# nianticlabs/mickey

Measured on AMD Instinct MI355X. Metric: image pairs/sec (540x720), higher is better.
Workload: dtype bf16

## Files before the change

### include/mickey_hip_dev.h

```cpp
#ifndef MICKEY_HIP_DEV_H
#define MICKEY_HIP_DEV_H

#ifdef __cplusplus
extern "C" {
#endif

int mk_gemm_set_tile(int mode);

int mk_attn_set_mode(int mode);

int mk_dev_mfma_sustained(float* scratch, int workgroups, int iters, int zero_operands, void* stream);

#ifdef __cplusplus
}
#endif
#endif
```

### mickey_amd/_native.py

```python
import ctypes
import os

import torch

from . import build as _build

MK_BF16, MK_F16, MK_F32 = 0, 1, 2
ACT_NONE, ACT_RELU, ACT_GELU = 0, 1, 2

_P, _I, _L, _F, _U = ctypes.c_void_p, ctypes.c_int, ctypes.c_longlong, ctypes.c_float, ctypes.c_ulonglong
_CODES = {"p": _P, "i": _I, "l": _L, "f": _F, "u": _U}

SIGNATURES = {
    "mk_version": ("i", ""),
    "mk_last_error": ("s", ""),
    "mk_preprocess_u8": ("i", "pliiipiip"),
    "mk_gemm": ("i", "pipippiiiiiiip"),
    "mk_gemm_grouped": ("i", "pilpilplpiliiiiiiip"),
    "mk_gemm_ls_residual": ("i", "pipipppiiiiip"),
    "mk_gemm_qkv": ("i", "pipippppiiiifip"),
    "mk_gemm_patch_embed": ("i", "pipipppiiiiip"),
    "mk_gemm_ls_residual_ln": ("i", "pipippppipppiiiiip"),
    "mk_gemm_patch_embed_ln": ("i", "pipipppppiiiiip"),
    "mk_cls_token_ln": ("i", "pppppiiiip"),
    "mk_recentre_split": ("i", "ppplilp"),
    "mk_gemm_ln": ("i", "pipipppfppiiiiiip"),
    "mk_gemm_qkv_ln": ("i", "pipipppfppppiiiifip"),
    "mk_im2col_patch14": ("i", "plliiiipiip"),
    "mk_cls_token": ("i", "pppiiip"),
    "mk_layernorm": ("i", "pippfpiipiiiiiiiiiip"),
    "mk_gemm_ln128": ("i", "pilpilppfpipiiiiiiip"),
    "mk_layernorm_planes": ("i", "pippfppifpiiiiiiiiipp"),
    "mk_flash_attn_fwd": ("i", "ppppiiiiiip"),
    "mk_bordered_rows": ("l", "iii"),
    "mk_conv3x3": ("i", "pliplipilplplpiliiiiiiip"),
    "mk_conv3x3_split": ("i", "pplipplipilplppiliiiiiiffpp"),
    "mk_split_planes": ("i", "plilfpplpp"),
    "mk_gemm_grouped_split": ("i", "ppilpilplppiliiiiiffpp"),
    "mk_posenc_add": ("i", "ppppiiiiiip"),
    "mk_linattn_work_floats": ("l", "iiii"),
    "mk_linattn_kv": ("i", "pppiiiip"),
    "mk_linattn_apply": ("i", "pppiiiiiip"),
    "mk_head_tails": ("i", "pppppppppppiiiiiiiififp"),
    "mk_dual_softmax_work_floats": ("l", "iiii"),
    "mk_dual_softmax": ("i", "ppppfifppppiiiip"),
    "mk_dual_softmax_split_work_floats": ("l", "iii"),
    "mk_dual_softmax_split": ("i", "ppppfifppppiiiip"),
    "mk_sinkhorn_work_floats": ("l", "iii"),
    "mk_sinkhorn": ("i", "ppppfippppiiiip"),
    "mk_dual_softmax_kf": ("i", "ppppfifppppiiiipip"),
    "mk_dual_softmax_split_kf": ("i", "ppppfifppppiiiipip"),
    "mk_sinkhorn_kf": ("i", "ppppfippppiiiipip"),
    "mk_mutual_nn": ("i", "ppppiiip"),
    "mk_dual_softmax_train_work_floats": ("l", "iiii"),
    "mk_dual_softmax_train": ("i", "ppppfppppppiiiiip"),
    "mk_dual_softmax_bwd_work_floats": ("l", "iiii"),
    "mk_dual_softmax_bwd": ("i", "ppppfpppppppppiiiiip"),
    "mk_exprace_topk_work_bytes": ("l", "iiil"),
    "mk_exprace_topk_state_bytes": ("l", "ii"),
    "mk_exprace_topk": ("i", "ppuupppppiiliip"),
    "mk_counter_add": ("i", "pup"),
    "mk_gather_backproject": ("i", "ppppppppppppiiiiip"),
    "mk_gather_backproject_kf": ("i", "ppppppppppppiiiiipip"),
    "mk_gather_backproject_bwd": ("i", "ppppppppppiiiiip"),
    "mk_ransac_hypotheses": ("i", "pppppuupfppppiiilp"),
    "mk_refine_pose": ("i", "pppppfiipppppppiiiip"),
    "mk_pose_finalize": ("i", "ppppip"),
    "mk_train_ransac_masks": ("i", "pppppuupfiipppiiilp"),
    "mk_reinforce_scatter": ("i", "ppppiiilp"),
    "mk_train_tail_fwd": ("i", "pppppppiiiifiifpppp"),
    "mk_train_tail_bwd": ("i", "pppppppiiiifiifppppppp"),
    "mk_train_aggregate_fwd": ("i", "pppiiififfppppp"),
    "mk_train_aggregate_bwd": ("i", "ppiiipp"),
}

DEV_SIGNATURES = {
    "mk_gemm_set_tile": ("i", "i"),
    "mk_attn_set_mode": ("i", "i"),
    "mk_dev_mfma_sustained": ("i", "piiip"),
}

_lib = None
_missing = set()


class MickeyHipError(RuntimeError):
    pass


def lib_path():
    return os.environ.get("MICKEY_HIP_LIB", _build.lib_path())


def load():
    global _lib
    if _lib is not None:
        return _lib
    path = lib_path()
    if not os.path.exists(path):
        raise MickeyHipError("libmickey_hip.so not found at %s -- build it with `python -m mickey_amd.build` "
                             "(mickey_amd has no CPU/ATen fallback)" % path)
    lib = ctypes.CDLL(path)
    for name, (res, args) in list(SIGNATURES.items()) + list(DEV_SIGNATURES.items()):
        try:
            fn = getattr(lib, name)
        except AttributeError:
            _missing.add(name)
            continue
        fn.restype = ctypes.c_char_p if res == "s" else _CODES[res]
        fn.argtypes = [_CODES[c] for c in args]
    _lib = lib
    return lib


def exported_symbols():
    return list(SIGNATURES)


def missing_symbols():
    load()
    return sorted(_missing)


def ptr(t):
    if t is None:
        return None
    if not t.is_cuda:
        raise MickeyHipError("expected a device tensor")
    return t.data_ptr()


def stream():
    return torch.cuda.current_stream().cuda_stream


def dtype_code(dt):
    if dt == torch.bfloat16:
        return MK_BF16
    if dt == torch.float16:
        return MK_F16
    if dt == torch.float32:
        return MK_F32
    raise MickeyHipError("unsupported low-precision dtype %s" % dt)


def call(name, *args):
    lib = load()
    if name in _missing:
        raise MickeyHipError("libmickey_hip.so does not export %s (stale build?)" % name)
    rc = getattr(lib, name)(*args)
    if rc != 0:
        raise MickeyHipError("%s failed (%d): %s" % (name, rc, lib.mk_last_error().decode()))


def query(name, *args):
    return getattr(load(), name)(*args)
```

### mickey_amd/csrc/mk_gemm.hip

```cpp
#include "mk_gemm_common.hpp"

namespace mk {
namespace gemm {
namespace {

template <typename T, int AMODE, int WMF, bool SP = false>
__global__ __launch_bounds__(256, 1) void gemm_kernel(GemmParams p) {
  using V8 = typename Lp<T>::V8;
  constexpr int NWM = 2, NWN = 2;
  constexpr int NW = NWM * NWN, BM = NWM * WMF * 16, BN = NWN * 64;
  constexpr int AJ = BM / 8 / NW, WJ = BN / 8 / NW;
  constexpr int A_BYTES = BM * 128, STAGE_BYTES = (BM + BN) * 128;
  constexpr int NS = WMF == 2 ? 3 : 2;
  constexpr int PIECES = AJ + WJ;
  extern __shared__ __attribute__((aligned(16))) char smem[];

  const int tid = threadIdx.x;
  const int lane = tid & 63;
  const int wave = __builtin_amdgcn_readfirstlane(tid >> 6);
  const int wm = wave / NWN, wn = wave % NWN;
  const int g = blockIdx.y;
  const int ntm = (p.M + BM - 1) / BM, ntn = (p.N + BN - 1) / BN;
  const int nk = p.K / BK;
  const int fr = lane & 15, fg = lane >> 4;

  const int id = xcd_remap(blockIdx.x, ntm * ntn);
  const int m0 = (id / ntn) * BM, n0 = (id % ntn) * BN;
  Stager<T, AMODE, NW, AJ, WJ, SP> st;
  st.init(p, g, m0, n0, wave, lane);
  st.issue(p, smem, smem + A_BYTES, 0);
  if (NS == 3 && nk > 1) st.issue(p, smem + STAGE_BYTES, smem + STAGE_BYTES + A_BYTES, 1);
  float2* lnp = (float2*)(smem + NS * STAGE_BYTES);
  if (AMODE == A_DENSE && p.ln_stats && tid < 2 * BM) ln_params_to_lds<BM, 2 * BM>(p, m0, tid, lnp, p.ln_shift_out != nullptr && n0 == 0);
  f32x4 acc[WMF][4];
#pragma unroll
  for (int i = 0; i < WMF; ++i)
#pragma unroll
    for (int j = 0; j < 4; ++j) acc[i][j] = f32x4{0.f, 0.f, 0.f, 0.f};
  int cur = 0, nxt = NS - 1;
  for (int kt = 0; kt < nk; ++kt) {
    if (NS == 3 && kt + 1 < nk) asm volatile("s_waitcnt vmcnt(%0)" ::"n"(PIECES) : "memory");
    else asm volatile("s_waitcnt vmcnt(0)" ::: "memory");
    asm volatile("s_waitcnt lgkmcnt(0)" ::: "memory");
    __builtin_amdgcn_s_barrier();
    char* nA = smem + nxt * STAGE_BYTES;
    if (kt + NS - 1 < nk) st.issue(p, nA, nA + A_BYTES, kt + NS - 1);
    const char* sA = smem + cur * STAGE_BYTES;
    const char* sW = sA + A_BYTES;
    cur = cur + 1 == NS ? 0 : cur + 1;
    nxt = nxt + 1 == NS ? 0 : nxt + 1;
    if constexpr (SP) {
      V8 wf[2][4], xf[2][WMF];
#pragma unroll
      for (int ks = 0; ks < 2; ++ks) {
#pragma unroll
        for (int i = 0; i < 4; ++i) {
          const int rw = wn * 64 + i * 16 + fr;
          wf[ks][i] = *(const V8*)(sW + rw * 128 + swz8(rw, ks * 4 + fg) * 16);
        }
#pragma unroll
        for (int i = 0; i < WMF; ++i) {
          const int rx = wm * (WMF * 16) + i * 16 + fr;
          xf[ks][i] = *(const V8*)(sA + rx * 128 + swz8(rx, ks * 4 + fg) * 16);
        }
      }
#pragma unroll
      for (int pr = 0; pr < 3; ++pr) {
        if (pr == 2 && p.npass == 2) break;
#pragma unroll
        for (int mi = 0; mi < WMF; ++mi)
#pragma unroll
          for (int ni = 0; ni < 4; ++ni) acc[mi][ni] = Lp<T>::mma16(wf[pr == 1][ni], xf[pr == 2][mi], acc[mi][ni]);
      }
    } else {
#pragma unroll
      for (int ks = 0; ks < 2; ++ks) {
        V8 wf[4], xf[WMF];
#pragma unroll
        for (int i = 0; i < 4; ++i) {
          const int rw = wn * 64 + i * 16 + fr;
          wf[i] = *(const V8*)(sW + rw * 128 + swz8(rw, ks * 4 + fg) * 16);
        }
#pragma unroll
        for (int i = 0; i < WMF; ++i) {
          const int rx = wm * (WMF * 16) + i * 16 + fr;
          xf[i] = *(const V8*)(sA + rx * 128 + swz8(rx, ks * 4 + fg) * 16);
        }
#pragma unroll
        for (int mi = 0; mi < WMF; ++mi)
#pragma unroll
          for (int ni = 0; ni < 4; ++ni) acc[mi][ni] = Lp<T>::mma16(wf[ni], xf[mi], acc[mi][ni]);
      }
    }
  }
  epilogue<T, WMF>(p, acc, m0, n0, wm, wn, lane, g, lnp);
}

template <typename T, int AMODE, int WMF, bool SP = false>
int launch_small(const GemmParams& p, int groups, hipStream_t st) {
  constexpr int BM = 32 * WMF;
  constexpr int LDS = (WMF == 2 ? 3 : 2) * (BM + 128) * 128 + BM * 8;
  static bool attr_done = false;
  if (!attr_done) {
    hipError_t e = hipFuncSetAttribute((const void*)gemm_kernel<T, AMODE, WMF, SP>, hipFuncAttributeMaxDynamicSharedMemorySize, LDS);
    if (e != hipSuccess) {
      mk_set_error("gemm: cannot reserve %d B of LDS: %s", LDS, hipGetErrorString(e));
      return MK_ERR_LAUNCH;
    }
    attr_done = true;
  }
  const int ntm = (p.M + BM - 1) / BM, ntn = (p.N + 127) / 128;
  hipLaunchKernelGGL((gemm_kernel<T, AMODE, WMF, SP>), dim3(ntm * ntn, groups, 1), dim3(256), LDS, st, p);
  MK_CHECK_LAUNCH();
  return MK_OK;
}

int g_num_cus = 0;
int g_band_m = 0;
int g_half_rows = 1;
int g_schedule = 0;

template <int AMODE>
int launch(const GemmParams& p, int groups, int dtype, hipStream_t st) {
  const long long big_tiles = (long long)((p.M + 255) / 256) * ((p.N + 255) / 256) * groups;
  bool big = p.N >= 256 && big_tiles >= 192;
  const long long plmax = p.npass > 1 ? (long long)max(max(p.pl1[0], p.pl1[1]), max(p.pl2[0], p.pl2[1])) / 2 : 0;
  const bool k_ok = p.K >= 2 * BK && (long long)p.M * p.lda + plmax < (1ll << 31) && (long long)p.N * p.ldw < (1ll << 31) &&
                    (AMODE == A_DENSE || bordered_rows(p.M / (p.H * p.Wd), p.H, p.Wd) * (p.C1 > p.C2 ? p.C1 : p.C2) + plmax < (1ll << 31));
  const bool ln_fold = p.ln_stats || p.xh;
  if (dtype == MK_F32) {
    MK_CHECK_ARG(!ln_fold, "gemm: the folded-LayerNorm epilogues exist for 16-bit operands only");
    return launch_f32(p, groups, AMODE, st);
  }
  int sched = g_schedule;
  if (sched == 0) sched = (big && k_ok) ? 7 : 1;
  if (!k_ok) sched = 1;
  if (sched == 7) return launch_pp64(p, groups, dtype, AMODE, st, g_band_m);
  const long long small_tiles = (long long)((p.M + 127) / 128) * ((p.N + 127) / 128) * groups;
  const bool half_rows = g_schedule == 2 || (g_schedule != 1 && g_half_rows && small_tiles < 2 * num_cus() && p.M > 64);
  if (p.npass > 1)
    return half_rows ? launch_small<_Float16, AMODE, 2, true>(p, groups, st) : launch_small<_Float16, AMODE, 4, true>(p, groups, st);
  if (half_rows) return dtype == MK_BF16 ? launch_small<__bf16, AMODE, 2>(p, groups, st) : launch_small<_Float16, AMODE, 2>(p, groups, st);
  return dtype == MK_BF16 ? launch_small<__bf16, AMODE, 4>(p, groups, st) : launch_small<_Float16, AMODE, 4>(p, groups, st);
}

int check_common(const GemmParams& p, int dtype) {
  MK_CHECK_ARG(dtype == MK_BF16 || dtype == MK_F16 || dtype == MK_F32, "gemm: dtype must be MK_BF16, MK_F16 or MK_F32");
  MK_CHECK_ARG(p.M > 0 && p.N > 0 && p.K > 0, "gemm: empty problem M=%d N=%d K=%d", p.M, p.N, p.K);
  const int kt = dtype == MK_F32 ? KT<float> : BK;
  MK_CHECK_ARG(p.K % kt == 0, "gemm: K=%d must be a multiple of %d", p.K, kt);
  MK_CHECK_ARG(p.N % 4 == 0, "gemm: N=%d must be a multiple of 4", p.N);
  MK_CHECK_ARG(p.ldw % 8 == 0 && p.ldw >= p.K, "gemm: ldw=%d must be >= K and a multiple of 8", p.ldw);
  MK_CHECK_ARG(p.A && p.W, "gemm: null operand");
  return MK_OK;
}

}

int num_cus() {
  if (g_num_cus == 0) {
    int dev = 0, n = 0;
    if (hipGetDevice(&dev) != hipSuccess || hipDeviceGetAttribute(&n, hipDeviceAttributeMultiprocessorCount, dev) != hipSuccess || n <= 0)
      n = 256;
    g_num_cus = n;
  }
  return g_num_cus;
}

}
}

using namespace mk;
using namespace mk::gemm;

extern "C" {

int mk_gemm_set_tile(int mode) {
  if (mode >= 400 && mode < 464) {
    g_band_m = mode - 400;
    return MK_OK;
  }
  if (mode >= 464 && mode < 496) {
    g_band_m = -(mode - 464);
    return MK_OK;
  }
  if (mode == 500 || mode == 501) {
    g_half_rows = mode - 500;
    return MK_OK;
  }
  if (mode >= 600 && mode <= 602) {
    g_pp64_persist = mode - 600;
    return MK_OK;
  }
  MK_CHECK_ARG(mode == 0 || mode == 1 || mode == 2 || mode == 7,
               "mk_gemm_set_tile: unknown mode %d (0 automatic, 1 128x128, 2 64x128, 7 8-wave ping-pong)", mode);
  g_schedule = mode;
  return MK_OK;
}

int mk_gemm(const void* A, int lda, const void* W, int ldw, const float* bias, void* out, int ldc, int M, int N, int K,
            int act, int out_is_f32, int dtype, mk_stream_t stream) {
  GemmParams p = {};
  p.A = A; p.W = W; p.M = M; p.N = N; p.K = K; p.lda = lda; p.ldw = ldw;
  p.epi = MK_EPI_STORE; p.act = act; p.bias = bias; p.ldc = ldc;
  if (out_is_f32) p.out_f32 = (float*)out; else p.out_lp = out;
  if (int e = check_common(p, dtype)) return e;
  MK_CHECK_ARG(lda % 8 == 0 && lda >= K && ldc % 4 == 0 && ldc >= N && out, "mk_gemm: bad lda/ldc/out");
  return launch<A_DENSE>(p, 1, dtype, (hipStream_t)stream);
}

int mk_gemm_grouped(const void* A, int lda, long long strideA, const void* W, int ldw, long long strideW, const float* bias,
                    long long strideBias, void* out, int ldc, long long strideOut, int groups, int M, int N, int K, int act,
                    int out_is_f32, int dtype, mk_stream_t stream) {
  GemmParams p = {};
  p.A = A; p.W = W; p.M = M; p.N = N; p.K = K; p.lda = lda; p.ldw = ldw;
  p.strideA_g = strideA; p.strideW_g = strideW; p.strideBias_g = strideBias; p.strideOut_g = strideOut;
  p.epi = MK_EPI_STORE; p.act = act; p.bias = bias; p.ldc = ldc;
  if (out_is_f32) p.out_f32 = (float*)out; else p.out_lp = out;
  if (int e = check_common(p, dtype)) return e;
  MK_CHECK_ARG(groups > 0 && lda % 8 == 0 && lda >= K && ldc % 4 == 0 && ldc >= N && out, "mk_gemm_grouped: bad args");
  return launch<A_DENSE>(p, groups, dtype, (hipStream_t)stream);
}

int mk_gemm_ls_residual(const void* A, int lda, const void* W, int ldw, const float* bias, const float* gamma, float* x,
                        int ldx, int M, int N, int K, int dtype, mk_stream_t stream) {
  GemmParams p = {};
  p.A = A; p.W = W; p.M = M; p.N = N; p.K = K; p.lda = lda; p.ldw = ldw;
  p.epi = MK_EPI_LS_RESIDUAL; p.bias = bias; p.gamma = gamma; p.out_f32 = x; p.ldc = ldx;
  if (int e = check_common(p, dtype)) return e;
  MK_CHECK_ARG(bias && gamma && x && lda % 8 == 0 && lda >= K && ldx % 4 == 0 && ldx >= N, "mk_gemm_ls_residual: bad args");
  return launch<A_DENSE>(p, 1, dtype, (hipStream_t)stream);
}

int mk_gemm_qkv(const void* A, int lda, const void* W, int ldw, const float* bias, void* q, void* k, void* vt, int nimg,
                int ntok, int ntok_pad, int heads, float qscale, int dtype, mk_stream_t stream) {
  GemmParams p = {};
  const int D = heads * 64;
  p.A = A; p.W = W; p.M = nimg * ntok; p.N = 3 * D; p.K = D; p.lda = lda; p.ldw = ldw;
  p.epi = MK_EPI_QKV; p.bias = bias; p.q = q; p.k = k; p.vt = vt;
  p.ntok = ntok; p.ntok_pad = ntok_pad; p.heads = heads; p.qscale = qscale;
  if (int e = check_common(p, dtype)) return e;
  MK_CHECK_ARG(bias && q && k && vt && ntok_pad % 64 == 0 && ntok_pad >= ntok && lda % 8 == 0 && lda >= D, "mk_gemm_qkv: bad args");
  return launch<A_DENSE>(p, 1, dtype, (hipStream_t)stream);
}

int mk_gemm_patch_embed(const void* A, int lda, const void* W, int ldw, const float* bias, const float* pos, float* x,
                        int nimg, int npatch, int D, int K, int dtype, mk_stream_t stream) {
  GemmParams p = {};
  p.A = A; p.W = W; p.M = nimg * npatch; p.N = D; p.K = K; p.lda = lda; p.ldw = ldw;
  p.epi = MK_EPI_PATCH; p.bias = bias; p.pos = pos; p.npatch = npatch; p.out_f32 = x; p.ldc = D;
  if (int e = check_common(p, dtype)) return e;
  MK_CHECK_ARG(bias && pos && x && lda % 8 == 0 && lda >= K, "mk_gemm_patch_embed: bad args");
  return launch<A_DENSE>(p, 1, dtype, (hipStream_t)stream);
}


static int ln_consumer_args(GemmParams& p, const float* colsum, const float* stats, float eps, float* shift_out, const char* who) {
  MK_CHECK_ARG(colsum && stats && p.bias, "%s: colsum, stats and bias are required", who);
  MK_CHECK_ARG(p.lda == p.K, "%s: the normalised width is K: lda must equal K", who);
  p.ln_colsum = colsum; p.ln_stats = stats; p.ln_nslot = p.K / 64; p.ln_eps = eps; p.ln_shift_out = shift_out;
  return MK_OK;
}

int mk_gemm_ln(const void* A, int lda, const void* W, int ldw, const float* bias, const float* colsum, const float* stats,
               float eps, float* shift_out, void* out, int ldc, int M, int N, int K, int act, int dtype, mk_stream_t stream) {
  GemmParams p = {};
  p.A = A; p.W = W; p.M = M; p.N = N; p.K = K; p.lda = lda; p.ldw = ldw;
  p.epi = MK_EPI_STORE; p.act = act; p.bias = bias; p.ldc = ldc; p.out_lp = out;
  if (int e = check_common(p, dtype)) return e;
  MK_CHECK_ARG(lda % 8 == 0 && ldc % 4 == 0 && ldc >= N && out && (act == MK_ACT_NONE || act == MK_ACT_GELU), "mk_gemm_ln: bad args");
  if (int e = ln_consumer_args(p, colsum, stats, eps, shift_out, "mk_gemm_ln")) return e;
  return launch<A_DENSE>(p, 1, dtype, (hipStream_t)stream);
}

int mk_gemm_qkv_ln(const void* A, int lda, const void* W, int ldw, const float* bias, const float* colsum, const float* stats,
                   float eps, float* shift_out, void* q, void* k, void* vt, int nimg, int ntok, int ntok_pad, int heads,
                   float qscale, int dtype, mk_stream_t stream) {
  GemmParams p = {};
  const int D = heads * 64;
  p.A = A; p.W = W; p.M = nimg * ntok; p.N = 3 * D; p.K = D; p.lda = lda; p.ldw = ldw;
  p.epi = MK_EPI_QKV; p.bias = bias; p.q = q; p.k = k; p.vt = vt;
  p.ntok = ntok; p.ntok_pad = ntok_pad; p.heads = heads; p.qscale = qscale;
  if (int e = check_common(p, dtype)) return e;
  MK_CHECK_ARG(q && k && vt && ntok_pad % 64 == 0 && ntok_pad >= ntok && lda % 8 == 0, "mk_gemm_qkv_ln: bad args");
  if (int e = ln_consumer_args(p, colsum, stats, eps, shift_out, "mk_gemm_qkv_ln")) return e;
  return launch<A_DENSE>(p, 1, dtype, (hipStream_t)stream);
}

int mk_gemm_ls_residual_ln(const void* A, int lda, const void* W, int ldw, const float* bias, const float* gamma, void* xh,
                           void* xl, int ldxs, float* stats, const float* shift_in, float* x_f32_out, int ldx, int M, int N,
                           int K, int dtype, mk_stream_t stream) {
  GemmParams p = {};
  p.A = A; p.W = W; p.M = M; p.N = N; p.K = K; p.lda = lda; p.ldw = ldw;
  p.epi = MK_EPI_LS_RESIDUAL; p.bias = bias; p.gamma = gamma; p.out_f32 = x_f32_out; p.ldc = ldx;
  p.xh = xh; p.xl = xl; p.ldxs = ldxs; p.stats_out = stats; p.nslot_out = N / 64; p.ln_shift_in = shift_in;
  if (int e = check_common(p, dtype)) return e;
  MK_CHECK_ARG(bias && gamma && lda % 8 == 0 && lda >= K, "mk_gemm_ls_residual_ln: bad args");
  MK_CHECK_ARG(xh && xl && N % 64 == 0 && ldxs % 8 == 0 && ldxs >= N, "mk_gemm_ls_residual_ln: xh / xl / N %% 64");
  MK_CHECK_ARG(x_f32_out ? (ldx % 4 == 0 && ldx >= N) : stats != nullptr, "mk_gemm_ls_residual_ln: stats, or x_f32_out with ldx");
  return launch<A_DENSE>(p, 1, dtype, (hipStream_t)stream);
}

int mk_gemm_patch_embed_ln(const void* A, int lda, const void* W, int ldw, const float* bias, const float* pos, void* xh,
                           void* xl, float* stats, int nimg, int npatch, int D, int K, int dtype, mk_stream_t stream) {
  GemmParams p = {};
  p.A = A; p.W = W; p.M = nimg * npatch; p.N = D; p.K = K; p.lda = lda; p.ldw = ldw;
  p.epi = MK_EPI_PATCH; p.bias = bias; p.pos = pos; p.npatch = npatch; p.ldc = D;
  p.xh = xh; p.xl = xl; p.ldxs = D; p.stats_out = stats; p.nslot_out = D / 64;
  if (int e = check_common(p, dtype)) return e;
  MK_CHECK_ARG(bias && pos && lda % 8 == 0 && lda >= K, "mk_gemm_patch_embed_ln: bad args");
  MK_CHECK_ARG(xh && xl && stats && D % 64 == 0, "mk_gemm_patch_embed_ln: xh / xl / stats / D %% 64");
  return launch<A_DENSE>(p, 1, dtype, (hipStream_t)stream);
}

long long mk_bordered_rows(int nimg, int H, int Wd) { return bordered_rows(nimg, H, Wd); }

int mk_conv3x3(const void* in1, long long stride_in1, int C1, const void* in2, long long stride_in2, int C2, const void* W,
               int ldw, long long strideW, const float* bias, long long strideBias, const void* resid, long long strideResid,
               void* out, int Cout, long long strideOut, int groups, int nimg, int H, int Wd, int act, int out_kind, int dtype,
               mk_stream_t stream) {
  GemmParams p = {};
  p.A = in1; p.A2 = in2; p.W = W;
  p.M = nimg * H * Wd; p.N = Cout; p.K = 9 * C1 + (in2 ? C2 : 0);
  p.ldw = ldw; p.strideA_g = stride_in1; p.strideA2_g = stride_in2; p.strideW_g = strideW;
  p.strideBias_g = strideBias; p.strideOut_g = strideOut;
  p.H = H; p.Wd = Wd; p.C1 = C1; p.C2 = in2 ? C2 : 0;
  p.epi = MK_EPI_STORE; p.act = act; p.bias = bias; p.ldc = Cout; p.resid_lp = resid; p.strideResid_g = strideResid;
  if (out_kind == MK_CONV_OUT_F32) p.out_f32 = (float*)out; else p.out_lp = out;
  p.bord_out = out_kind == MK_CONV_OUT_BORDERED;
  if (int e = check_common(p, dtype)) return e;
  MK_CHECK_ARG(C1 % (dtype == MK_F32 ? 32 : BK) == 0 && (!in2 || C2 % (dtype == MK_F32 ? 32 : BK) == 0),
               "mk_conv3x3: channel counts must be multiples of the K tile (%d)", dtype == MK_F32 ? 32 : BK);
  MK_CHECK_ARG(out && groups > 0 && nimg > 0 && H > 0 && Wd > 0 && out_kind >= 0 && out_kind <= 2, "mk_conv3x3: bad args");
  return launch<A_CONV3>(p, groups, dtype, (hipStream_t)stream);
}

namespace {
__global__ __launch_bounds__(256) void split_planes_kernel(const float* __restrict__ src, long long rows, int cols4, long long ld_src4,
                                                           float scale, uint2* __restrict__ hi, uint2* __restrict__ lo, long long ld_dst4, int* sat_flag) {
  const long long t = blockIdx.x * 256LL + threadIdx.x;
  if (t >= rows * cols4) return;
  const long long r = t / cols4;
  const int c = (int)(t - r * cols4);
  const long long i = r * ld_dst4 + c;
  const f32x4 x = __builtin_nontemporal_load((const f32x4*)src + r * ld_src4 + c) * scale;
  f16x4 h, l;
#pragma unroll
  for (int e = 0; e < 4; ++e) {
    const float v = sat16(x[e], sat_flag);
    h[e] = (_Float16)v;
    l[e] = (_Float16)(v - (float)h[e]);
  }
  hi[i] = __builtin_bit_cast(uint2, h);
  lo[i] = __builtin_bit_cast(uint2, l);
}
}

int mk_split_planes(const float* src, long long rows, int cols, long long ld_src, float scale, void* hi, void* lo,
                    long long ld_dst, int* sat_flag, mk_stream_t stream) {
  MK_CHECK_ARG(src && hi && lo && rows > 0 && cols > 0 && cols % 4 == 0 && ld_src % 4 == 0 && ld_dst % 4 == 0 && ld_src >= cols &&
                   ld_dst >= cols, "mk_split_planes: cols / ld_src / ld_dst must be multiples of 4 and ld >= cols");
  MK_CHECK_ARG((((uintptr_t)src | (uintptr_t)hi * 2 | (uintptr_t)lo * 2) & 15) == 0, "mk_split_planes: src must be 16-byte, planes 8-byte aligned");
  const long long n4 = rows * (cols / 4);
  hipLaunchKernelGGL(split_planes_kernel, dim3((unsigned)((n4 + 255) / 256)), dim3(256), 0, (hipStream_t)stream, src, rows, cols / 4,
                     ld_src / 4, scale, (uint2*)hi, (uint2*)lo, ld_dst / 4, sat_flag);
  MK_CHECK_LAUNCH();
  return MK_OK;
}

static int split_source(const void* hi, const void* lo, const void*& base, unsigned (&pl)[2], const char* who) {
  const uintptr_t h = (uintptr_t)hi, l = (uintptr_t)lo, b = h < l ? h : l;
  MK_CHECK_ARG((h - b) < (1ull << 31) && (l - b) < (1ull << 31) && ((h | l) & 15) == 0,
               "%s: the (hi, lo) planes of a source must be 16-byte aligned and lie within 2 GiB of each other", who);
  base = (const void*)b;
  pl[0] = (unsigned)(h - b);
  pl[1] = (unsigned)(l - b);
  return MK_OK;
}

int mk_gemm_grouped_split(const void* A_hi, const void* A_lo, int lda, long long strideA, const void* W, int ldw, long long strideW,
                          const float* bias, long long strideBias, void* out, void* out_lo, int ldc, long long strideOut, int groups,
                          int M, int N, int K, int act, float acc_scale, float plane_scale, int* sat_flag, mk_stream_t stream) {
  GemmParams p = {};
  MK_CHECK_ARG(A_hi && A_lo, "mk_gemm_grouped_split: null plane");
  if (int e = split_source(A_hi, A_lo, p.A, p.pl1, "mk_gemm_grouped_split")) return e;
  p.W = W; p.M = M; p.N = N; p.K = 2 * K; p.lda = lda; p.ldw = ldw;
  p.npass = 3; p.acc_scale = acc_scale;
  p.strideA_g = strideA; p.strideW_g = strideW; p.strideBias_g = strideBias; p.strideOut_g = strideOut;
  p.epi = MK_EPI_STORE; p.act = act; p.bias = bias; p.ldc = ldc;
  if (out_lo) { p.out_lp = out; p.out_lo = out_lo; p.plane_scale = plane_scale; p.sat_flag = sat_flag; } else { p.out_f32 = (float*)out; }
  if (int e = check_common(p, MK_F16)) return e;
  MK_CHECK_ARG(out && groups > 0 && K % 32 == 0 && lda % 8 == 0 && lda >= K && ldc % 4 == 0 && ldc >= N,
               "mk_gemm_grouped_split: bad args (K must be a multiple of 32)");
  return launch<A_DENSE>(p, groups, MK_F16, (hipStream_t)stream);
}

int mk_conv3x3_split(const void* in1_hi, const void* in1_lo, long long stride_in1, int C1, const void* in2_hi, const void* in2_lo,
                     long long stride_in2, int C2, const void* W, int ldw, long long strideW, const float* bias,
                     long long strideBias, void* out, void* out_lo, int Cout, long long strideOut, int groups, int nimg, int H,
                     int Wd, int act, int out_bordered, float acc_scale, float plane_scale, int* sat_flag, mk_stream_t stream) {
  GemmParams p = {};
  const bool hi_only = in1_hi && !in1_lo;
  MK_CHECK_ARG(in1_hi && (hi_only ? (!in2_hi && !in2_lo) : (!in2_hi == !in2_lo)),
               "mk_conv3x3_split: every source needs both planes (in1_lo == NULL = an all-zero lo plane: then without in2)");
  if (int e = split_source(in1_hi, hi_only ? in1_hi : in1_lo, p.A, p.pl1, "mk_conv3x3_split")) return e;
  if (in2_hi) {
    if (int e = split_source(in2_hi, in2_lo, p.A2, p.pl2, "mk_conv3x3_split")) return e;
  }
  p.W = W;
  p.npass = hi_only ? 2 : 3; p.acc_scale = acc_scale;
  p.M = nimg * H * Wd; p.N = Cout; p.K = 2 * (9 * C1 + (in2_hi ? C2 : 0));
  p.ldw = ldw; p.strideA_g = stride_in1; p.strideA2_g = stride_in2; p.strideW_g = strideW;
  p.strideBias_g = strideBias; p.strideOut_g = strideOut;
  p.H = H; p.Wd = Wd; p.C1 = C1; p.C2 = in2_hi ? C2 : 0;
  p.epi = MK_EPI_STORE; p.act = act; p.bias = bias; p.ldc = Cout;
  if (out_lo) { p.out_lp = out; p.out_lo = out_lo; p.plane_scale = plane_scale; p.sat_flag = sat_flag; } else { p.out_f32 = (float*)out; }
  p.bord_out = out_bordered ? 1 : 0;
  if (int e = check_common(p, MK_F16)) return e;
  MK_CHECK_ARG(C1 % 32 == 0 && (!in2_hi || C2 % 32 == 0), "mk_conv3x3_split: channel counts must be multiples of 32");
  MK_CHECK_ARG(out && groups > 0 && nimg > 0 && H > 0 && Wd > 0, "mk_conv3x3_split: bad args");
  return launch<A_CONV3>(p, groups, MK_F16, (hipStream_t)stream);
}

}
```

### mickey_amd/csrc/mk_gemm_common.hpp

```cpp
#pragma once
#include "mk_common.hpp"

namespace mk {
namespace gemm {

constexpr int BK = 64;
template <typename T> constexpr int EPC = 16 / (int)sizeof(T);
template <typename T> constexpr int KT = 128 / (int)sizeof(T);

enum AMode { A_DENSE = 0, A_CONV3 = 1 };

struct GemmParams {
  const void* A;
  const void* A2;
  const void* W;
  int M, N, K, lda, ldw;
  long long strideA_g, strideA2_g, strideW_g;
  int H, Wd, C1, C2;
  int bord_out;
  unsigned pl1[2], pl2[2];
  int npass;
  float acc_scale;
  void* out_lo;
  float plane_scale;
  int* sat_flag;
  int epi;
  int act;
  const float* bias;
  const float* gamma;
  long long strideBias_g;
  float* out_f32;
  void* out_lp;
  int ldc;
  long long strideOut_g;
  const void* resid_lp;
  long long strideResid_g;
  void* q;
  void* k;
  void* vt;
  int ntok, ntok_pad, heads;
  float qscale;
  const float* pos;
  int npatch;
  void* xh;
  void* xl;
  int ldxs;
  float* stats_out;
  int nslot_out;
  const float* ln_stats;
  const float* ln_colsum;
  int ln_nslot;
  float ln_eps;
  float* ln_shift_out;
  const float* ln_shift_in;
};

__device__ __forceinline__ void quad_stats(const f32x4& x, float& s, float& q) {
  s = x[0];
  s += x[1];
  s += x[2];
  s += x[3];
  q = __builtin_fmaf(x[0], x[0], 0.0f);
  q = __builtin_fmaf(x[1], x[1], q);
  q = __builtin_fmaf(x[2], x[2], q);
  q = __builtin_fmaf(x[3], x[3], q);
}

__device__ __forceinline__ float row16_sum(float v) {
#define MK_DPP_ADD(ctrl) v += __builtin_bit_cast(float, __builtin_amdgcn_update_dpp(0, __builtin_bit_cast(int, v), ctrl, 0xf, 0xf, true))
  MK_DPP_ADD(0xB1);
  MK_DPP_ADD(0x4E);
  MK_DPP_ADD(0x141);
  MK_DPP_ADD(0x140);
#undef MK_DPP_ADD
  return v;
}

typedef __attribute__((ext_vector_type(4))) unsigned u32x4;
struct LnRowLoads16 {
  u32x4 v[4];
  __device__ __forceinline__ void issue(const GemmParams& p, int m0, int tid) {
    const int wave = tid >> 6, lane = tid & 63;
    const long long last = (long long)p.M * 128 - 16;
#pragma unroll
    for (int j = 0; j < 4; ++j) {
      long long off = ((long long)(m0 + wave * 32 + j * 8) * 128) + lane * 16;
      off = off < last ? off : last;
      const char* a = (const char*)p.ln_stats + off;
      asm volatile("global_load_dwordx4 %0, %1, off" : "=v"(v[j]) : "v"(a) : "memory");
    }
  }
  template <int YOUNGER>
  __device__ __forceinline__ void finish(const GemmParams& p, int tid, float2* prm, int m0 = 0, bool publish = false) {
    asm volatile("s_waitcnt vmcnt(%4)" : "+v"(v[0]), "+v"(v[1]), "+v"(v[2]), "+v"(v[3]) : "n"(YOUNGER) : "memory");
    const int wave = tid >> 6, lane = tid & 63;
#pragma unroll
    for (int j = 0; j < 4; ++j) {
      const f32x4 f = __builtin_bit_cast(f32x4, v[j]);
      float s = f[0] + f[2], q = f[1] + f[3];
#define MK_DPP_ADD(x, ctrl) x += __builtin_bit_cast(float, __builtin_amdgcn_update_dpp(0, __builtin_bit_cast(int, x), ctrl, 0xf, 0xf, true))
      MK_DPP_ADD(s, 0xB1);  MK_DPP_ADD(q, 0xB1);
      MK_DPP_ADD(s, 0x4E);  MK_DPP_ADD(q, 0x4E);
      MK_DPP_ADD(s, 0x141); MK_DPP_ADD(q, 0x141);
#undef MK_DPP_ADD
      const double mean = (double)s * (1.0 / 1024.0);
      double var = (double)q * (1.0 / 1024.0) - mean * mean;
      var = var > 0.0 ? var : 0.0;
      const float rstd = 1.0f / sqrtf((float)var + p.ln_eps);
      if ((lane & 7) == 0) {
        const int r = wave * 32 + j * 8 + (lane >> 3);
        prm[r] = make_float2(rstd, -(float)mean * rstd);
        if (publish && m0 + r < p.M) p.ln_shift_out[m0 + r] = (float)mean;
      }
    }
  }
};

struct LnRowDma16 {
  template <int J0>
  __device__ __forceinline__ static void issue(const GemmParams& p, int m0, int wave, int lane, char* stage_lds) {
    const long long last = (long long)p.M * 128 - 16;
#pragma unroll
    for (int j = J0; j < J0 + 2; ++j) {
      const long long base = (long long)(m0 + wave * 32 + j * 8) * 128;
      long long off = base + lane * 16;
      off = off < last ? off : last;
      glds16_sv((const char*)p.ln_stats, (unsigned)off, stage_lds + (wave * 2 + (j - J0)) * 1024);
    }
  }
  template <int J0>
  __device__ __forceinline__ static void finish(const GemmParams& p, int wave, int lane, float2* prm, const char* stage_lds, int m0,
                                                bool publish) {
#pragma unroll
    for (int j = J0; j < J0 + 2; ++j) {
      const f32x4 f = *(const f32x4*)(stage_lds + (wave * 2 + (j - J0)) * 1024 + lane * 16);
      float s = f[0] + f[2], q = f[1] + f[3];
#define MK_DPP_ADD(x, ctrl) x += __builtin_bit_cast(float, __builtin_amdgcn_update_dpp(0, __builtin_bit_cast(int, x), ctrl, 0xf, 0xf, true))
      MK_DPP_ADD(s, 0xB1);  MK_DPP_ADD(q, 0xB1);
      MK_DPP_ADD(s, 0x4E);  MK_DPP_ADD(q, 0x4E);
      MK_DPP_ADD(s, 0x141); MK_DPP_ADD(q, 0x141);
#undef MK_DPP_ADD
      const double mean = (double)s * (1.0 / 1024.0);
      double var = (double)q * (1.0 / 1024.0) - mean * mean;
      var = var > 0.0 ? var : 0.0;
      const float rstd = 1.0f / sqrtf((float)var + p.ln_eps);
      if ((lane & 7) == 0) {
        const int r = wave * 32 + j * 8 + (lane >> 3);
        prm[r] = make_float2(rstd, -(float)mean * rstd);
        if (publish && m0 + r < p.M) p.ln_shift_out[m0 + r] = (float)mean;
      }
    }
  }
};

struct ShiftLoad {
  float v;
  __device__ __forceinline__ void issue(const GemmParams& p, int m0, int tid, int BM) {
    v = 0.f;
    if (p.ln_shift_in && tid < BM) {
      int m = m0 + tid;
      m = m < p.M ? m : p.M - 1;
      const float* a = p.ln_shift_in + m;
      asm volatile("global_load_dword %0, %1, off" : "=v"(v) : "v"(a) : "memory");
    }
  }
  template <int YOUNGER>
  __device__ __forceinline__ void finish(int tid, int BM, float* shl) {
    if constexpr (YOUNGER >= 0)
      asm volatile("s_waitcnt vmcnt(%1)" : "+v"(v) : "n"(YOUNGER) : "memory");
    else
      asm volatile("" : "+v"(v) : : "memory");
    if (tid < BM) shl[tid] = v;
  }
};

template <int BM, int NT>
__device__ __forceinline__ void ln_params_to_lds(const GemmParams& p, int m0, int tid, float2* prm, bool publish = false) {
  static_assert(NT == 2 * BM, "two threads per row");
  const int r = tid >> 1, h = tid & 1;
  int m = m0 + r;
  m = m < p.M ? m : p.M - 1;
  const float2* st = (const float2*)p.ln_stats + (long long)m * p.ln_nslot;
  float s, q;
  if (p.ln_nslot <= 16) {
    float2 v[8];
#pragma unroll
    for (int j = 0; j < 8; ++j) v[j] = 8 * h + j < p.ln_nslot ? st[8 * h + j] : make_float2(0.f, 0.f);
    const float s01 = v[0].x + v[1].x, s23 = v[2].x + v[3].x, s45 = v[4].x + v[5].x, s67 = v[6].x + v[7].x;
    const float q01 = v[0].y + v[1].y, q23 = v[2].y + v[3].y, q45 = v[4].y + v[5].y, q67 = v[6].y + v[7].y;
    s = (s01 + s23) + (s45 + s67);
    q = (q01 + q23) + (q45 + q67);
  } else {
    const int per = (p.ln_nslot + 1) >> 1;
    const int lo = h * per, hi = min(p.ln_nslot, lo + per);
    s = q = 0.f;
    for (int i0 = lo; i0 < hi; i0 += 8) {
      float2 v[8];
#pragma unroll
      for (int j = 0; j < 8; ++j) v[j] = i0 + j < hi ? st[i0 + j] : make_float2(0.f, 0.f);
#pragma unroll
      for (int j = 0; j < 8; ++j) {
        s += v[j].x;
        q += v[j].y;
      }
    }
  }
  s += __shfl_xor(s, 1, 64);
  q += __shfl_xor(q, 1, 64);
  const double invn = 1.0 / (64.0 * p.ln_nslot);
  const double mean = (double)s * invn;
  double var = (double)q * invn - mean * mean;
  var = var > 0.0 ? var : 0.0;
  const float rstd = 1.0f / sqrtf((float)var + p.ln_eps);
  if (h == 0) {
    prm[r] = make_float2(rstd, -(float)mean * rstd);
    if (publish && m0 + r < p.M) p.ln_shift_out[m0 + r] = (float)mean;
  }
}

template <typename T>
__device__ __forceinline__ T to_lp(float v) { return (T)v; }

template <typename T>
__device__ __forceinline__ f32x4 unpack4(uint2 u);
template <>
__device__ __forceinline__ f32x4 unpack4<__bf16>(uint2 u) {
  return f32x4{__builtin_bit_cast(float, u.x << 16), __builtin_bit_cast(float, u.x & 0xffff0000u),
               __builtin_bit_cast(float, u.y << 16), __builtin_bit_cast(float, u.y & 0xffff0000u)};
}
template <>
__device__ __forceinline__ f32x4 unpack4<_Float16>(uint2 u) {
  const f16x4 h = __builtin_bit_cast(f16x4, u);
  return f32x4{(float)h[0], (float)h[1], (float)h[2], (float)h[3]};
}
template <>
__device__ __forceinline__ f32x4 unpack4<float>(uint2) { return f32x4{0.f, 0.f, 0.f, 0.f}; }
template <typename T>
__device__ __forceinline__ uint2 pack4(f32x4 v) {
  typename Lp<T>::V4 o;
#pragma unroll
  for (int e = 0; e < 4; ++e) o[e] = to_lp<T>(v[e]);
  if constexpr (sizeof(T) == 2) return __builtin_bit_cast(uint2, o);
  else return uint2{0u, 0u};
}

__device__ __forceinline__ int vperm(int t) { return (t & ~12) | ((t & 4) << 1) | ((t & 8) >> 1); }

template <typename T, int AMODE, int NW, int AJ, int WJ, bool SP = false>
struct Stager {
  const T* A;
  const T* A2;
  const T* wrow[WJ];
  long long aoff[AJ];
  int wave, srow, sp;

  __device__ __forceinline__ void init(const GemmParams& p, int g, int m0, int n0, int wave_, int lane) {
    wave = wave_;
    srow = lane >> 3;
    sp = lane & 7;
    A = (const T*)p.A + (long long)g * p.strideA_g;
    A2 = p.A2 ? (const T*)p.A2 + (long long)g * p.strideA2_g : nullptr;
    const T* W = (const T*)p.W + (long long)g * p.strideW_g;
#pragma unroll
    for (int j = 0; j < WJ; ++j) {
      const int r = (wave * WJ + j) * 8 + srow;
      int n = n0 + r;
      n = n < p.N ? n : p.N - 1;
      wrow[j] = W + (long long)n * p.ldw + swz8(r, sp) * EPC<T>;
    }
#pragma unroll
    for (int j = 0; j < AJ; ++j) {
      const int r = (wave * AJ + j) * 8 + srow;
      int m = m0 + r;
      m = m < p.M ? m : p.M - 1;
      const int c = swz8(r, sp);
      if (AMODE == A_DENSE) aoff[j] = SP ? (long long)m * p.lda + (c & 3) * EPC<T> + (long long)(((c >> 2) ? p.pl1[1] : p.pl1[0]) / sizeof(T))
                                         : (long long)m * p.lda + c * EPC<T>;
      else aoff[j] = bordered_row(m, p.H, p.Wd);
    }
  }

  __device__ __forceinline__ void issue(const GemmParams& p, char* sA, char* sW, int kt) const {
    const int k0 = kt * KT<T>;
    const int ka = SP ? kt * (KT<T> / 2) : k0;
    if (AMODE == A_DENSE) {
#pragma unroll
      for (int j = 0; j < AJ; ++j) glds16(A + aoff[j] + ka, sA + (wave * AJ + j) * 1024);
    } else {
      const int kc = 9 * p.C1;
      const T* const s1 = A;
      const T* const s2 = A2;
      const T* src;
      int cs, c0, shift = 0;
      unsigned plh, pll;
      if (ka < kc) {
        const int tap = ka / p.C1;
        c0 = ka - tap * p.C1;
        shift = (tap / 3 - 1) * (p.Wd + 1) + tap % 3 - 1;
        src = s1;
        cs = p.C1;
        plh = p.pl1[0];
        pll = p.pl1[1];
      } else {
        c0 = ka - kc;
        src = s2;
        cs = p.C2;
        plh = p.pl2[0];
        pll = p.pl2[1];
      }
#pragma unroll
      for (int j = 0; j < AJ; ++j) {
        const int r = (wave * AJ + j) * 8 + srow;
        const int c = swz8(r, sp);
        if (SP) glds16(src + (aoff[j] + shift) * cs + c0 + (c & 3) * EPC<T> + (long long)(((c >> 2) ? pll : plh) / sizeof(T)), sA + (wave * AJ + j) * 1024);
        else glds16(src + (aoff[j] + shift) * cs + c0 + c * EPC<T>, sA + (wave * AJ + j) * 1024);
      }
    }
#pragma unroll
    for (int j = 0; j < WJ; ++j) glds16(wrow[j] + k0, sW + (wave * WJ + j) * 1024);
  }
};

template <typename T, int WMF, int EPI, int ACT, bool HAS_BIAS, bool LN = false, bool SPLIT = false>
__device__ __forceinline__ void epilogue_impl(const GemmParams& p, f32x4 (&acc)[WMF][4], int m0, int n0, int wm, int wn, int lane,
                                              int g, const float2* lnp = nullptr) {
  using V4 = typename Lp<T>::V4;
  const int fr = lane & 15, fg = lane >> 4;
  const float* bias = HAS_BIAS ? p.bias + (long long)g * p.strideBias_g : nullptr;
  const int nb = n0 + wn * 64 + fg * 4;
  f32x4 bv[4], cs[4];
#pragma unroll
  for (int ni = 0; ni < 4; ++ni) {
    const int n = nb + ni * 16;
    bv[ni] = (HAS_BIAS && n < p.N) ? *(const f32x4*)(bias + n) : f32x4{0.f, 0.f, 0.f, 0.f};
    cs[ni] = (LN && n < p.N) ? *(const f32x4*)(p.ln_colsum + n) : f32x4{0.f, 0.f, 0.f, 0.f};
  }
  const bool fin = SPLIT && EPI == MK_EPI_LS_RESIDUAL && p.out_f32 != nullptr;
#pragma unroll
  for (int mi = 0; mi < WMF; ++mi) {
    const int m = m0 + wm * (WMF * 16) + mi * 16 + fr;
    if (SPLIT) {
      const bool mok = m < p.M;
      long long xrow = m;
      int tok1 = 0;
      if (EPI == MK_EPI_PATCH) {
        const int img = m / p.npatch;
        tok1 = 1 + (m - img * p.npatch);
        xrow = (long long)img * (p.npatch + 1) + tok1;
      }
      const float shv = (EPI == MK_EPI_LS_RESIDUAL && p.ln_shift_in && mok) ? p.ln_shift_in[m] : 0.f;
      float s4[4] = {0.f, 0.f, 0.f, 0.f}, q4[4] = {0.f, 0.f, 0.f, 0.f};
#pragma unroll
      for (int ni = 0; ni < 4; ++ni) {
        const int n = nb + ni * 16;
        if (!(mok && n < p.N)) continue;
        f32x4 v = acc[mi][ni] + bv[ni];
        T* ph = (T*)p.xh + xrow * p.ldxs + n;
        T* pl = (T*)p.xl + xrow * p.ldxs + n;
        if (EPI == MK_EPI_LS_RESIDUAL) {
          const f32x4 gm = *(const f32x4*)(p.gamma + n);
          const V4 h = *(const V4*)ph, l = *(const V4*)pl;
          f32x4 r;
#pragma unroll
          for (int e = 0; e < 4; ++e) r[e] = (float)h[e] + (float)l[e];
          r += gm * v;
          r -= shv;
          v = r;
        } else {
          v += *(const f32x4*)(p.pos + (long long)tok1 * p.N + n);
        }
        if (fin) {
          *(f32x4*)(p.out_f32 + xrow * p.ldc + n) = v;
          continue;
        }
        V4 oh, ol;
#pragma unroll
        for (int e = 0; e < 4; ++e) {
          oh[e] = to_lp<T>(v[e]);
          ol[e] = to_lp<T>(v[e] - (float)oh[e]);
        }
        quad_stats(v, s4[ni], q4[ni]);
        *(V4*)ph = oh;
        *(V4*)pl = ol;
      }
#pragma unroll
      for (int ni = 0; ni < 4; ++ni) {
        s4[ni] += __shfl_xor(s4[ni], 16, 64);
        q4[ni] += __shfl_xor(q4[ni], 16, 64);
        s4[ni] += __shfl_xor(s4[ni], 32, 64);
        q4[ni] += __shfl_xor(q4[ni], 32, 64);
      }
      const float ssum = (s4[0] + s4[1]) + (s4[2] + s4[3]), qsum = (q4[0] + q4[1]) + (q4[2] + q4[3]);
      if (!fin && fg == 0 && mok && n0 + wn * 64 < p.N)
        ((float2*)p.stats_out)[xrow * p.nslot_out + ((n0 + wn * 64) >> 6)] = make_float2(ssum, qsum);
      continue;
    }
    if (m >= p.M) continue;
    float2 prm = make_float2(1.f, 0.f);
    if (LN) prm = lnp[wm * (WMF * 16) + mi * 16 + fr];
    int img = 0, tok = 0;
    if (EPI == MK_EPI_QKV) {
      img = m / p.ntok;
      tok = m - img * p.ntok;
    } else if (EPI == MK_EPI_PATCH) {
      img = m / p.npatch;
      tok = m - img * p.npatch;
    }
    const long long brow = (EPI == MK_EPI_STORE && p.H > 0) ? bordered_row(m, p.H, p.Wd) : (long long)m;
#pragma unroll
    for (int ni = 0; ni < 4; ++ni) {
      const int n = nb + ni * 16;
      if (n >= p.N) continue;
      f32x4 v = acc[mi][ni];
      if (EPI == MK_EPI_STORE && p.npass > 1) {
        const float sc = p.acc_scale;
#pragma unroll
        for (int e = 0; e < 4; ++e) v[e] *= sc;
      }
      if (LN) v = v * prm.x + (cs[ni] * prm.y + bv[ni]);
      else if (HAS_BIAS) v += bv[ni];
      if (EPI == MK_EPI_STORE) {
        if (p.resid_lp) {
          const V4 r = *(const V4*)((const T*)p.resid_lp + (long long)g * p.strideResid_g + brow * p.ldc + n);
#pragma unroll
          for (int e = 0; e < 4; ++e) v[e] += (float)r[e];
        }
        if (ACT == MK_ACT_RELU) {
#pragma unroll
          for (int e = 0; e < 4; ++e) v[e] = fmaxf(v[e], 0.f);
        } else if (ACT == MK_ACT_GELU) {
          v = gelu_erf4(v);
        }
        if (p.out_lo) {
          const float ps = p.plane_scale;
          f16x4 oh, ol;
#pragma unroll
          for (int e = 0; e < 4; ++e) {
            const float sv = sat16(v[e] * ps, p.sat_flag);
            oh[e] = (_Float16)sv;
            ol[e] = (_Float16)(sv - (float)oh[e]);
          }
          const long long o = (long long)g * p.strideOut_g + (p.bord_out ? brow : (long long)m) * p.ldc + n;
          *(f16x4*)((_Float16*)p.out_lp + o) = oh;
          *(f16x4*)((_Float16*)p.out_lo + o) = ol;
        } else if (p.out_f32) {
          *(f32x4*)(p.out_f32 + (long long)g * p.strideOut_g + (p.bord_out ? brow : (long long)m) * p.ldc + n) = v;
        } else {
          V4 o;
#pragma unroll
          for (int e = 0; e < 4; ++e) o[e] = to_lp<T>(v[e]);
          *(V4*)((T*)p.out_lp + (long long)g * p.strideOut_g + (p.bord_out ? brow : (long long)m) * p.ldc + n) = o;
        }
      } else if (EPI == MK_EPI_LS_RESIDUAL) {
        float* x = p.out_f32 + (long long)m * p.ldc + n;
        const f32x4 gm = *(const f32x4*)(p.gamma + n);
        f32x4 r = *(const f32x4*)x;
        r += gm * v;
        *(f32x4*)x = r;
      } else if (EPI == MK_EPI_PATCH) {
        const f32x4 pe = *(const f32x4*)(p.pos + (long long)(1 + tok) * p.N + n);
        *(f32x4*)(p.out_f32 + ((long long)img * (p.npatch + 1) + 1 + tok) * p.ldc + n) = v + pe;
      } else {
        const int D = p.heads * 64;
        const int which = n / D;
        const int rem = n - which * D;
        const int head = rem >> 6, d = rem & 63;
        const long long hb = (long long)img * p.heads + head;
        if (which == 2) {
          T* dst = (T*)p.vt + (hb * 64 + d) * p.ntok_pad + vperm(tok);
#pragma unroll
          for (int e = 0; e < 4; ++e) dst[(long long)e * p.ntok_pad] = to_lp<T>(v[e]);
        } else {
          if (which == 0) { const float qs = p.qscale; _Pragma("unroll") for (int e = 0; e < 4; ++e) v[e] *= qs; }
          V4 o;
#pragma unroll
          for (int e = 0; e < 4; ++e) o[e] = to_lp<T>(v[e]);
          T* base = (T*)(which == 0 ? p.q : p.k);
          *(V4*)(base + (hb * p.ntok_pad + tok) * 64 + d) = o;
        }
      }
    }
  }
}

template <typename T, int WMF>
__device__ __forceinline__ void epilogue(const GemmParams& p, f32x4 (&acc)[WMF][4], int m0, int n0, int wm, int wn, int lane,
                                         int g, const float2* lnp = nullptr) {
  if (p.xh) {
    if (p.epi == MK_EPI_PATCH) epilogue_impl<T, WMF, MK_EPI_PATCH, MK_ACT_NONE, true, false, true>(p, acc, m0, n0, wm, wn, lane, g);
    else epilogue_impl<T, WMF, MK_EPI_LS_RESIDUAL, MK_ACT_NONE, true, false, true>(p, acc, m0, n0, wm, wn, lane, g);
    return;
  }
  if (p.ln_stats) {
    if (p.epi == MK_EPI_QKV) epilogue_impl<T, WMF, MK_EPI_QKV, MK_ACT_NONE, true, true>(p, acc, m0, n0, wm, wn, lane, g, lnp);
    else if (p.act == MK_ACT_GELU) epilogue_impl<T, WMF, MK_EPI_STORE, MK_ACT_GELU, true, true>(p, acc, m0, n0, wm, wn, lane, g, lnp);
    else epilogue_impl<T, WMF, MK_EPI_STORE, MK_ACT_NONE, true, true>(p, acc, m0, n0, wm, wn, lane, g, lnp);
    return;
  }
  switch (p.epi) {
    case MK_EPI_LS_RESIDUAL: epilogue_impl<T, WMF, MK_EPI_LS_RESIDUAL, MK_ACT_NONE, true>(p, acc, m0, n0, wm, wn, lane, g); break;
    case MK_EPI_QKV: epilogue_impl<T, WMF, MK_EPI_QKV, MK_ACT_NONE, true>(p, acc, m0, n0, wm, wn, lane, g); break;
    case MK_EPI_PATCH: epilogue_impl<T, WMF, MK_EPI_PATCH, MK_ACT_NONE, true>(p, acc, m0, n0, wm, wn, lane, g); break;
    default:
      if (!p.bias) {
        if (p.act == MK_ACT_RELU) epilogue_impl<T, WMF, MK_EPI_STORE, MK_ACT_RELU, false>(p, acc, m0, n0, wm, wn, lane, g);
        else if (p.act == MK_ACT_GELU) epilogue_impl<T, WMF, MK_EPI_STORE, MK_ACT_GELU, false>(p, acc, m0, n0, wm, wn, lane, g);
        else epilogue_impl<T, WMF, MK_EPI_STORE, MK_ACT_NONE, false>(p, acc, m0, n0, wm, wn, lane, g);
      } else {
        if (p.act == MK_ACT_RELU) epilogue_impl<T, WMF, MK_EPI_STORE, MK_ACT_RELU, true>(p, acc, m0, n0, wm, wn, lane, g);
        else if (p.act == MK_ACT_GELU) epilogue_impl<T, WMF, MK_EPI_STORE, MK_ACT_GELU, true>(p, acc, m0, n0, wm, wn, lane, g);
        else epilogue_impl<T, WMF, MK_EPI_STORE, MK_ACT_NONE, true>(p, acc, m0, n0, wm, wn, lane, g);
      }
  }
}

template <typename T, int EPI, int ACT, bool HAS_BIAS, bool LN = false, bool SPLIT = false, bool FIN = false, bool CONV = false>
__device__ __forceinline__ void epilogue_lds_impl(const GemmParams& p, f32x4 (&acc)[8][4], char* wl0, char* wl1, int m0, int n0, int wm,
                                                  int wn, int lane, int g, const float2* lnp = nullptr) {
  using V4 = typename Lp<T>::V4;
  using V8 = typename Lp<T>::V8;
  const int fr = lane & 15, fg = lane >> 4;
  const float* bias = HAS_BIAS ? p.bias + (long long)g * p.strideBias_g : nullptr;
  const int nw = n0 + wn * 64;
  const int mw = m0 + wm * 128;
  int img0 = 0, tok0 = 0;
  if (EPI == MK_EPI_QKV) {
    img0 = mw / p.ntok;
    tok0 = mw - img0 * p.ntok;
  }
  auto img_tok = [&](int r, int& img, int& tok) {
    if (p.ntok >= 128) {
      const int t = tok0 + r;
      const bool wrap = t >= p.ntok;
      img = img0 + (wrap ? 1 : 0);
      tok = wrap ? t - p.ntok : t;
    } else {
      const int m = mw + r;
      img = m / p.ntok;
      tok = m - img * p.ntok;
    }
  };
  f32x4 bv[4], cs[4];
#pragma unroll
  for (int ni = 0; ni < 4; ++ni) {
    const int n = nw + fg * 4 + ni * 16;
    bv[ni] = (HAS_BIAS && n < p.N) ? *(const f32x4*)(bias + n) : f32x4{0.f, 0.f, 0.f, 0.f};
    cs[ni] = (LN && n < p.N) ? *(const f32x4*)(p.ln_colsum + n) : f32x4{0.f, 0.f, 0.f, 0.f};
  }
  float2 prm[8];
#pragma unroll
  for (int mi = 0; mi < 8; ++mi) prm[mi] = LN ? lnp[wm * 128 + mi * 16 + fr] : make_float2(1.f, 0.f);
  const bool lp_out = EPI == MK_EPI_QKV || (EPI == MK_EPI_STORE && !p.out_f32 && !p.out_lo);
  if (lp_out) {
    int which = 0, head = 0;
    if (EPI == MK_EPI_QKV) {
      const int D = p.heads * 64;
      which = nw / D;
      head = (nw - which * D) >> 6;
      if (which == 2) {
#pragma unroll
        for (int mi = 0; mi < 8; ++mi) {
          const int m = mw + mi * 16 + fr;
          if (m >= p.M) continue;
          int img, tok;
          img_tok(mi * 16 + fr, img, tok);
          const long long hb = (long long)img * p.heads + head;
#pragma unroll
          for (int ni = 0; ni < 4; ++ni) {
            const f32x4 v = LN ? acc[mi][ni] * prm[mi].x + (cs[ni] * prm[mi].y + bv[ni]) : acc[mi][ni] + bv[ni];
            T* dst = (T*)p.vt + (hb * 64 + ni * 16 + fg * 4) * p.ntok_pad + vperm(tok);
#pragma unroll
            for (int e = 0; e < 4; ++e) dst[(long long)e * p.ntok_pad] = to_lp<T>(v[e]);
          }
        }
        return;
      }
    }
    const int rr = lane >> 3, c = lane & 7;
    const int n = nw + c * 8;
    const bool bord = CONV && p.bord_out;
    BorderedRow bw;
    if (bord) bw.init(mw + rr, p.H, p.Wd);
#pragma unroll
    for (int h = 0; h < 2; ++h) {
#pragma unroll
      for (int mq = 0; mq < 4; ++mq) {
        const int mi = h * 4 + mq;
        const int r = mi * 16 + fr;
        char* wrow = (mq < 2 ? wl0 : wl1) + ((mq & 1) * 16 + fr) * 128;
        const long long rrow = (CONV && p.resid_lp) ? bordered_row(min(mw + r, p.M - 1), p.H, p.Wd) : 0;
#pragma unroll
        for (int ni = 0; ni < 4; ++ni) {
          f32x4 v = acc[mi][ni];
          if (LN) v = v * prm[mi].x + (cs[ni] * prm[mi].y + bv[ni]);
          else if (HAS_BIAS) v += bv[ni];
          if (EPI == MK_EPI_QKV) {
            if (which == 0) { const float qs = p.qscale; _Pragma("unroll") for (int e = 0; e < 4; ++e) v[e] *= qs; }
          } else {
            if (CONV && p.resid_lp) {
              const int m = mw + r, n2 = nw + fg * 4 + ni * 16;
              if (m < p.M && n2 < p.N) {
                const V4 rs = *(const V4*)((const T*)p.resid_lp + (long long)g * p.strideResid_g + rrow * p.ldc + n2);
#pragma unroll
                for (int e = 0; e < 4; ++e) v[e] += (float)rs[e];
              }
            }
            if (ACT == MK_ACT_RELU) {
#pragma unroll
              for (int e = 0; e < 4; ++e) v[e] = fmaxf(v[e], 0.f);
            } else if (ACT == MK_ACT_GELU) {
              v = gelu_erf4(v);
            }
          }
          V4 o;
#pragma unroll
          for (int e = 0; e < 4; ++e) o[e] = to_lp<T>(v[e]);
          const int cc = ni * 2 + (fg >> 1);
          *(V4*)(wrow + ((cc ^ (fr & 7)) << 4) + (fg & 1) * 8) = o;
        }
      }
#pragma unroll
      for (int i8 = 0; i8 < 8; ++i8) {
        const int it = h * 8 + i8;
        const int r = it * 8 + rr;
        const int m = mw + r;
        const V8 val = *(const V8*)((i8 < 4 ? wl0 : wl1) + ((i8 & 3) * 8 + rr) * 128 + ((c ^ (rr & 7)) << 4));
        const int extra = bord ? bw.extra : 0;
        if (bord) bw.step(8, p.H, p.Wd);
        if (m >= p.M || n >= p.N) continue;
        T* dst;
        if (EPI == MK_EPI_QKV) {
          int img, tok;
          img_tok(r, img, tok);
          dst = (T*)(which == 0 ? p.q : p.k) + (((long long)img * p.heads + head) * p.ntok_pad + tok) * 64 + c * 8;
        } else {
          dst = (T*)p.out_lp + (long long)g * p.strideOut_g + ((long long)m + extra) * p.ldc + n;
        }
        if (n + 8 <= p.N) {
          *(V8*)dst = val;
        } else {
          V4 lo;
#pragma unroll
          for (int e = 0; e < 4; ++e) lo[e] = val[e];
          *(V4*)dst = lo;
        }
      }
    }
  } else {
    const int rr = lane >> 4, c = lane & 15;
    const int n = nw + c * 4;
    f32x4 gm = f32x4{0.f, 0.f, 0.f, 0.f};
    if (EPI == MK_EPI_LS_RESIDUAL && n < p.N) gm = *(const f32x4*)(p.gamma + n);
    f32x4 bvd = f32x4{0.f, 0.f, 0.f, 0.f};
    if (SPLIT && HAS_BIAS && n < p.N) bvd = *(const f32x4*)(bias + n);
    f32x4 xr[2][SPLIT ? 1 : 16];
    uint2 xh[2][SPLIT ? 16 : 1], xl[2][SPLIT ? 16 : 1];
    const unsigned lane_off = (unsigned)rr * (unsigned)p.ldxs + (unsigned)n;
    unsigned lane_off_st = lane_off;
    asm volatile("" : "+v"(lane_off_st));
    auto plane_row = [&](void* plane, int half, int it) -> T* {
      return (T*)plane + (long long)(mw + half * 64 + it * 4) * p.ldxs;
    };
    __amdgpu_buffer_rsrc_t rs_h, rs_l;
    unsigned voff_b = 0;
    if constexpr (SPLIT && EPI == MK_EPI_LS_RESIDUAL && sizeof(T) == 2) {
      rs_h = __builtin_amdgcn_make_buffer_rsrc(p.xh, 0, 0x7fffffff, 0x00020000);
      rs_l = __builtin_amdgcn_make_buffer_rsrc(p.xl, 0, 0x7fffffff, 0x00020000);
      voff_b = lane_off * 2u;
    }
    auto soff_b = [&](int half, int it) -> unsigned {
      return (unsigned)(mw + half * 64 + it * 4) * (unsigned)p.ldxs * 2u;
    };
    typedef unsigned u32x2_t __attribute__((ext_vector_type(2)));
    auto preload = [&](int half, int it0 = 0, int it1 = 16) {
      if (EPI != MK_EPI_LS_RESIDUAL) return;
#pragma unroll
      for (int it = 0; it < 16; ++it) {
        if (it < it0 || it >= it1) continue;
        const int m = mw + half * 64 + it * 4 + rr;
        const bool ok = SPLIT || (m < p.M && n < p.N);
        if constexpr (SPLIT && EPI == MK_EPI_LS_RESIDUAL && sizeof(T) == 2) {
          const u32x2_t a = __builtin_amdgcn_raw_buffer_load_b64(rs_h, voff_b, soff_b(half, it), 0);
          const u32x2_t b = __builtin_amdgcn_raw_buffer_load_b64(rs_l, voff_b, soff_b(half, it), 0);
          xh[half][it] = uint2{a[0], a[1]};
          xl[half][it] = uint2{b[0], b[1]};
        } else if (SPLIT) {
          xh[half][it] = ok ? *(const uint2*)(plane_row(p.xh, half, it) + lane_off) : uint2{0u, 0u};
          xl[half][it] = ok ? *(const uint2*)(plane_row(p.xl, half, it) + lane_off) : uint2{0u, 0u};
        } else {
          xr[half][it] = ok ? *(const f32x4*)(p.out_f32 + (long long)m * p.ldc + n) : f32x4{0.f, 0.f, 0.f, 0.f};
        }
      }
    };
    auto stageq = [&](int half, int sub) {
#pragma unroll
      for (int m2 = 0; m2 < 2; ++m2) {
        const int mi = sub * 2 + m2;
        const int r = mi * 16 + fr;
        char* wrow = (m2 == 0 ? wl0 : wl1) + fr * 256;
        const long long rrow = (CONV && p.resid_lp) ? bordered_row(min(mw + half * 64 + r, p.M - 1), p.H, p.Wd) : 0;
#pragma unroll
        for (int ni = 0; ni < 4; ++ni) {
          f32x4 v = acc[half * 4 + mi][ni];
          if (EPI == MK_EPI_STORE && p.npass > 1) {
            const float sc = p.acc_scale;
#pragma unroll
            for (int e = 0; e < 4; ++e) v[e] *= sc;
          }
          if (HAS_BIAS && !SPLIT) v += bv[ni];
          if (EPI == MK_EPI_STORE) {
            if (CONV && p.resid_lp) {
              const int m = mw + half * 64 + r, nn = nw + fg * 4 + ni * 16;
              if (m < p.M && nn < p.N) {
                const V4 rs = *(const V4*)((const T*)p.resid_lp + (long long)g * p.strideResid_g + rrow * p.ldc + nn);
#pragma unroll
                for (int e = 0; e < 4; ++e) v[e] += (float)rs[e];
              }
            }
            if (ACT == MK_ACT_RELU) {
#pragma unroll
              for (int e = 0; e < 4; ++e) v[e] = fmaxf(v[e], 0.f);
            } else if (ACT == MK_ACT_GELU) {
              v = gelu_erf4(v);
            }
          }
          const int cw = ni * 4 + fg;
          *(f32x4*)(wrow + ((cw ^ fr) << 4)) = v;
        }
      }
    };
    constexpr bool fin = FIN;
    auto emit_row = [&](long long xrow, T* dh, T* dl, f32x4 x, bool ok, unsigned soff = 0xffffffffu) {
      float ssum = 0.f, qsum = 0.f;
      if (ok) {
        const uint2 oh = pack4<T>(x);
        const uint2 ol = pack4<T>(x - unpack4<T>(oh));
        quad_stats(x, ssum, qsum);
        if constexpr (SPLIT && EPI == MK_EPI_LS_RESIDUAL && sizeof(T) == 2) {
          __builtin_amdgcn_raw_buffer_store_b64(u32x2_t{oh.x, oh.y}, rs_h, voff_b, soff, 0);
          __builtin_amdgcn_raw_buffer_store_b64(u32x2_t{ol.x, ol.y}, rs_l, voff_b, soff, 0);
        } else {
          *(uint2*)dh = oh;
          *(uint2*)dl = ol;
        }
      }
      ssum = row16_sum(ssum);
      qsum = row16_sum(qsum);
      if (ok && c == 0) ((float2*)p.stats_out)[xrow * p.nslot_out + (nw >> 6)] = make_float2(ssum, qsum);
    };
    auto drain = [&](int half, int it0 = 0, int it1 = 16) {
      const bool bordf = CONV && p.bord_out;
      BorderedRow bwf;
      if (bordf) bwf.init(mw + half * 64 + it0 * 4 + rr, p.H, p.Wd);
#pragma unroll
      for (int it = 0; it < 16; ++it) {
        if (it < it0 || it >= it1) continue;
        const int r = it * 4 + rr;
        const int m = mw + half * 64 + r;
        const int extraf = bordf ? bwf.extra : 0;
        if (bordf) bwf.step(4, p.H, p.Wd);
        f32x4 val = *(const f32x4*)(((it & 4) ? wl1 : wl0) + ((it & 3) * 4 + rr) * 256 + ((c ^ ((it & 3) * 4 + rr)) << 4));
        if (SPLIT) val += bvd;
        const bool ok = SPLIT || (m < p.M && n < p.N);
        if (!ok) continue;
        if (EPI == MK_EPI_LS_RESIDUAL) {
          f32x4 x;
          if (SPLIT) {
            x = unpack4<T>(xh[half][it]) + unpack4<T>(xl[half][it]);
          } else {
            x = xr[half][it];
          }
          x += gm * val;
          if (SPLIT) x -= ((const float*)lnp)[wm * 128 + half * 64 + r];
          if (!SPLIT || fin) {
            if (ok) *(f32x4*)(p.out_f32 + (long long)m * p.ldc + n) = x;
          } else {
            if constexpr (sizeof(T) == 2) emit_row(m, nullptr, nullptr, x, ok, soff_b(half, it));
            else emit_row(m, plane_row(p.xh, half, it) + lane_off_st, plane_row(p.xl, half, it) + lane_off_st, x, ok);
          }
        } else if (EPI == MK_EPI_PATCH) {
          const int mc = ok ? m : 0;
          const int img = mc / p.npatch, tok = mc - img * p.npatch;
          const long long xrow = (long long)img * (p.npatch + 1) + 1 + tok;
          f32x4 x = val;
          if (ok) x += *(const f32x4*)(p.pos + (long long)(1 + tok) * p.N + n);
          if (SPLIT) emit_row(xrow, (T*)p.xh + xrow * p.ldxs + n, (T*)p.xl + xrow * p.ldxs + n, x, ok);
          else if (ok) *(f32x4*)(p.out_f32 + xrow * p.ldc + n) = x;
        } else if (EPI == MK_EPI_STORE && p.out_lo) {
          const float ps = p.plane_scale;
          f16x4 oh, ol;
#pragma unroll
          for (int e = 0; e < 4; ++e) {
            const float sv = sat16(val[e] * ps, p.sat_flag);
            oh[e] = (_Float16)sv;
            ol[e] = (_Float16)(sv - (float)oh[e]);
          }
          const long long o = (long long)g * p.strideOut_g + ((long long)m + extraf) * p.ldc + n;
          *(f16x4*)((_Float16*)p.out_lp + o) = oh;
          *(f16x4*)((_Float16*)p.out_lo + o) = ol;
        } else {
          *(f32x4*)(p.out_f32 + (long long)g * p.strideOut_g + ((long long)m + extraf) * p.ldc + n) = val;
        }
      }
    };
    if (SPLIT && !FIN && EPI == MK_EPI_LS_RESIDUAL) {
      preload(0, 0, 16);
      stageq(0, 0);
      drain(0, 0, 8);
      preload(1, 0, 8);
      stageq(0, 1);
      drain(0, 8, 16);
      preload(1, 8, 16);
      stageq(1, 0);
      drain(1, 0, 8);
      stageq(1, 1);
      drain(1, 8, 16);
    } else {
      preload(0);
      stageq(0, 0);
      drain(0, 0, 8);
      stageq(0, 1);
      preload(1);
      drain(0, 8, 16);
      stageq(1, 0);
      drain(1, 0, 8);
      stageq(1, 1);
      drain(1, 8, 16);
    }
  }
}

template <typename T, int KIND, bool CONV = false, int BN = 256>
__device__ __forceinline__ void epilogue_lds(const GemmParams& p, f32x4 (&acc)[8][4], char* wl0, char* wl1, int m0, int n0, int wm,
                                             int wn, int lane, int g, const float2* lnp = nullptr) {
  if constexpr (KIND == 2 || KIND == 3) {
    const bool interior = m0 + 256 <= p.M && n0 + BN <= p.N;
    if (KIND == 3) {
      if (interior) epilogue_lds_impl<T, MK_EPI_LS_RESIDUAL, MK_ACT_NONE, true, false, true, true>(p, acc, wl0, wl1, m0, n0, wm, wn, lane, g, lnp);
      else epilogue_impl<T, 8, MK_EPI_LS_RESIDUAL, MK_ACT_NONE, true, false, true>(p, acc, m0, n0, wm, wn, lane, g);
    } else if (p.epi == MK_EPI_PATCH) {
      if (interior) epilogue_lds_impl<T, MK_EPI_PATCH, MK_ACT_NONE, true, false, true>(p, acc, wl0, wl1, m0, n0, wm, wn, lane, g);
      else epilogue_impl<T, 8, MK_EPI_PATCH, MK_ACT_NONE, true, false, true>(p, acc, m0, n0, wm, wn, lane, g);
    } else {
      if (interior) epilogue_lds_impl<T, MK_EPI_LS_RESIDUAL, MK_ACT_NONE, true, false, true, false>(p, acc, wl0, wl1, m0, n0, wm, wn, lane, g, lnp);
      else epilogue_impl<T, 8, MK_EPI_LS_RESIDUAL, MK_ACT_NONE, true, false, true>(p, acc, m0, n0, wm, wn, lane, g);
    }
  } else if constexpr (KIND == 1) {
#if defined(MK_LN_ABL) && MK_LN_ABL == 2
    constexpr bool LNE = false;
#else
    constexpr bool LNE = true;
#endif
    if (p.epi == MK_EPI_QKV) epilogue_lds_impl<T, MK_EPI_QKV, MK_ACT_NONE, true, LNE>(p, acc, wl0, wl1, m0, n0, wm, wn, lane, g, lnp);
    else if (p.act == MK_ACT_GELU) epilogue_lds_impl<T, MK_EPI_STORE, MK_ACT_GELU, true, LNE>(p, acc, wl0, wl1, m0, n0, wm, wn, lane, g, lnp);
    else epilogue_lds_impl<T, MK_EPI_STORE, MK_ACT_NONE, true, LNE>(p, acc, wl0, wl1, m0, n0, wm, wn, lane, g, lnp);
  } else {
    switch (CONV ? MK_EPI_STORE : p.epi) {
      case MK_EPI_LS_RESIDUAL: epilogue_lds_impl<T, MK_EPI_LS_RESIDUAL, MK_ACT_NONE, true>(p, acc, wl0, wl1, m0, n0, wm, wn, lane, g); break;
      case MK_EPI_QKV: epilogue_lds_impl<T, MK_EPI_QKV, MK_ACT_NONE, true>(p, acc, wl0, wl1, m0, n0, wm, wn, lane, g); break;
      case MK_EPI_PATCH: epilogue_lds_impl<T, MK_EPI_PATCH, MK_ACT_NONE, true>(p, acc, wl0, wl1, m0, n0, wm, wn, lane, g); break;
      default:
        if (!p.bias) {
          if (p.act == MK_ACT_RELU) epilogue_lds_impl<T, MK_EPI_STORE, MK_ACT_RELU, false, false, false, false, CONV>(p, acc, wl0, wl1, m0, n0, wm, wn, lane, g);
          else if (!CONV && p.act == MK_ACT_GELU) epilogue_lds_impl<T, MK_EPI_STORE, MK_ACT_GELU, false>(p, acc, wl0, wl1, m0, n0, wm, wn, lane, g);
          else epilogue_lds_impl<T, MK_EPI_STORE, MK_ACT_NONE, false, false, false, false, CONV>(p, acc, wl0, wl1, m0, n0, wm, wn, lane, g);
        } else {
          if (p.act == MK_ACT_RELU) epilogue_lds_impl<T, MK_EPI_STORE, MK_ACT_RELU, true, false, false, false, CONV>(p, acc, wl0, wl1, m0, n0, wm, wn, lane, g);
          else if (!CONV && p.act == MK_ACT_GELU) epilogue_lds_impl<T, MK_EPI_STORE, MK_ACT_GELU, true>(p, acc, wl0, wl1, m0, n0, wm, wn, lane, g);
          else epilogue_lds_impl<T, MK_EPI_STORE, MK_ACT_NONE, true, false, false, false, CONV>(p, acc, wl0, wl1, m0, n0, wm, wn, lane, g);
        }
    }
  }
}

__device__ __forceinline__ void pp_tile_coords(int id, int ntm, int ntn, int PP_GM, int& tm, int& tn) {
  if (PP_GM < 0) {
    const int ng = -PP_GM;
    const int grp = id / (ntm * ng);
    const int rem = id - grp * (ntm * ng);
    const int gn = min(ng, ntn - grp * ng);
    tm = rem / gn;
    tn = grp * ng + rem - tm * gn;
    return;
  }
  const int band = id / (PP_GM * ntn);
  const int rem = id - band * (PP_GM * ntn);
  const int gm = min(PP_GM, ntm - band * PP_GM);
  tm = band * PP_GM + rem % gm;
  tn = rem / gm;
}

int num_cus();
extern int g_pp64_persist;
int launch_pp64(const GemmParams& p, int groups, int dtype, int amode, hipStream_t st, int band_m);
int launch_f32(const GemmParams& p, int groups, int amode, hipStream_t st);

}
}
```

### mickey_amd/csrc/mk_gemm_pp64.hip

```cpp
#include <type_traits>

#include "mk_gemm_common.hpp"

namespace mk {
namespace gemm {
int g_pp64_persist = 2;
namespace {

template <typename T, int AMODE, int KIND, bool PERSIST = false, bool SP = false, bool SP2 = false>
__global__ __launch_bounds__(512, 2) void gemm_pp64_kernel(GemmParams p, int band_m) {
  static_assert(!SP2 || SP, "SP2 is a form of the split-operand kernel");
  static_assert(!PERSIST || AMODE == A_DENSE, "the persistent tile loop is built for dense operands");
  static_assert(!SP || (KIND == 0 && !PERSIST && sizeof(T) == 2), "split operands: plain epilogues, one tile per workgroup");
  constexpr int BKA = SP ? BK / 2 : BK;
  using V8 = typename Lp<T>::V8;
  constexpr int WMF = 8, BM = 256, BN = 256;
  constexpr int A_BYTES = BM * 128, STAGE_BYTES = (BM + BN) * 128;
  constexpr int LN_STAGE_OFF = 2 * STAGE_BYTES + 256 * 8;
  extern __shared__ __attribute__((aligned(16))) char smem[];

  const int tid0 = threadIdx.x;
  const int wave = __builtin_amdgcn_readfirstlane(tid0 >> 6);
  int lane = tid0 & 63, tid = tid0;
  auto refresh_lane = [&]() {
    if constexpr (PERSIST) {
      asm volatile("v_mbcnt_lo_u32_b32 %0, -1, 0\n\tv_mbcnt_hi_u32_b32 %0, -1, %0" : "=v"(lane));
      tid = wave * 64 + lane;
    }
  };
  const int wm = wave >> 2, wn = wave & 3;
  const int g = blockIdx.y;
  const int ntm = (p.M + BM - 1) / BM, ntn = (p.N + BN - 1) / BN;
  const int nk = p.K / BK;

  const T* A = (const T*)p.A + (long long)g * p.strideA_g;
  const T* A2 = p.A2 ? (const T*)p.A2 + (long long)g * p.strideA2_g : nullptr;
  const T* W = (const T*)p.W + (long long)g * p.strideW_g;
  int srow = lane >> 3, sp = lane & 7;
  const int ntiles = ntm * ntn;
  auto tile_origin = [&](int id, int& mm, int& nn) {
    int tm, tn;
    pp_tile_coords(xcd_remap(id, ntiles), ntm, ntn, band_m, tm, tn);
    mm = tm * BM;
    nn = tn * BN;
  };
  int bid = blockIdx.x;
  int m0, n0;
  tile_origin(bid, m0, n0);
  unsigned woff[4], aoff[4], aoff2[4];
  auto set_woff = [&](int nn0) {
#pragma unroll
    for (int j = 0; j < 4; ++j) {
      const int rw = (wave * 4 + j) * 8 + srow;
      int n = nn0 + rw;
      n = n < p.N ? n : p.N - 1;
      woff[j] = ((unsigned)n * (unsigned)p.ldw + swz8(rw, sp) * 8) * (unsigned)sizeof(T);
    }
  };
  auto set_aoff = [&](int mm0) {
#pragma unroll
    for (int j = 0; j < 4; ++j) {
      const int ra = wm * 128 + (wn * 4 + j) * 8 + srow;
      int m = mm0 + ra;
      m = m < p.M ? m : p.M - 1;
      const int c = swz8(ra, sp);
      const unsigned cc = SP ? (unsigned)(c & 3) : (unsigned)c;
      const bool lo = SP && (c >> 2) != 0;
      const unsigned pb1 = !SP ? 0u : (lo ? p.pl1[1] : p.pl1[0]), pb2 = !SP ? 0u : (lo ? p.pl2[1] : p.pl2[0]);
      if (AMODE == A_DENSE) {
        aoff[j] = ((unsigned)m * (unsigned)p.lda + cc * 8) * (unsigned)sizeof(T) + pb1;
        aoff2[j] = 0;
      } else {
        const unsigned br = (unsigned)bordered_row(m, p.H, p.Wd);
        aoff[j] = (br * (unsigned)p.C1 + cc * 8) * (unsigned)sizeof(T) + pb1;
        aoff2[j] = (br * (unsigned)p.C2 + cc * 8) * (unsigned)sizeof(T) + pb2;
      }
    }
  };
  set_woff(n0);
  set_aoff(m0);
  auto dma_w1 = [&](int s, int j) {
    glds16_sv(W + s * BK, woff[j], smem + (s & 1) * STAGE_BYTES + A_BYTES + (wave * 4 + j) * 1024);
  };
  const int ntap = A2 ? 10 : 9;
  const T* cbase = AMODE == A_DENSE ? A : A - (long long)(p.Wd + 2) * p.C1;
  int cleft = p.C1, ctap = 0;
  auto conv_advance = [&]() {
    cleft -= BKA;
    const bool wrap = cleft == 0;
    ctap += wrap ? 1 : 0;
    const int ty = (ctap * 11) >> 5, tx = ctap - 3 * ty;
    const T* tapbase = ctap < 9 ? A + (long long)((ty - 1) * (p.Wd + 1) + tx - 1) * p.C1 : A2;
    cbase = wrap ? tapbase : cbase + BKA;
    cleft = wrap ? (ctap < 9 ? p.C1 : p.C2) : cleft;
  };
  auto dma_a1 = [&](int s, int j) {
    char* dst = smem + (s & 1) * STAGE_BYTES + (wm * 16 + wn * 4 + j) * 1024;
    if (AMODE == A_DENSE) {
      glds16_sv(A + s * BKA, aoff[j], dst);
    } else {
      glds16_sv(cbase, ctap < 9 ? aoff[j] : aoff2[j], dst);
    }
  };
  auto dma_w = [&](int s) {
#pragma unroll
    for (int j = 0; j < 4; ++j) dma_w1(s, j);
  };
  auto dma_a = [&](int s) {
#pragma unroll
    for (int j = 0; j < 4; ++j) dma_a1(s, j);
    if (AMODE != A_DENSE) conv_advance();
  };

  int fr = lane & 15, fg = lane >> 4;
  auto derive_lane = [&]() {
    srow = lane >> 3;
    sp = lane & 7;
    fr = lane & 15;
    fg = lane >> 4;
  };
  auto load_w = [&](V8* wf, int par, int h) {
    const char* sW = smem + par * STAGE_BYTES + A_BYTES;
#pragma unroll
    for (int i = 0; i < 4; ++i) {
      const int rw = wn * 64 + i * 16 + fr;
      wf[i] = *(const V8*)(sW + rw * 128 + swz8(rw, h * 4 + fg) * 16);
    }
  };
  auto load_x = [&](V8* xf, int par, int h) {
    const char* sA = smem + par * STAGE_BYTES;
#pragma unroll
    for (int i = 0; i < WMF; ++i) {
      const int rx = wm * 128 + i * 16 + fr;
      xf[i] = *(const V8*)(sA + rx * 128 + swz8(rx, h * 4 + fg) * 16);
    }
  };
  auto load_frags = [&](V8* wf, V8* xf, int par, int h) {
    load_w(wf, par, h);
    load_x(xf, par, h);
  };
  f32x4 acc[WMF][4];
  auto zero_acc = [&]() {
#pragma unroll
    for (int i = 0; i < WMF; ++i)
#pragma unroll
      for (int j = 0; j < 4; ++j) acc[i][j] = f32x4{0.f, 0.f, 0.f, 0.f};
  };
  if constexpr (!PERSIST) zero_acc();
  auto mfma32 = [&](const V8* wf, const V8* xf, auto dma, int s, auto first) {
    constexpr bool DMA = decltype(dma)::value;
    constexpr bool FIRST = decltype(first)::value;
    __builtin_amdgcn_s_setprio(1);
    __builtin_amdgcn_sched_barrier(0);
#pragma unroll
    for (int q = 0; q < 32; ++q) {
      const int mi = q >> 2, ni = q & 3;
      acc[mi][ni] = Lp<T>::mma16(wf[ni], xf[mi], FIRST ? f32x4{0.f, 0.f, 0.f, 0.f} : acc[mi][ni]);
      if (DMA && (q & 7) == 3) {
        __builtin_amdgcn_sched_barrier(0);
        dma_a1(s, q >> 3);
        __builtin_amdgcn_sched_barrier(0);
      }
    }
    __builtin_amdgcn_sched_barrier(0);
    __builtin_amdgcn_s_setprio(0);
    if (DMA && AMODE != A_DENSE) conv_advance();
  };
  auto bar = [&]() {
    asm volatile("s_waitcnt lgkmcnt(0)" ::: "memory");
    __builtin_amdgcn_s_barrier();
  };
  using Yes = std::integral_constant<bool, true>;
  using No = std::integral_constant<bool, false>;
  V8 wf[4], xf[WMF];
  V8 wfl[SP ? 4 : 1];
  auto stage0 = [&](int kt, auto next1, auto next2, int sw, int sa, auto first) {
    if constexpr (SP && SP2) {
      bar();
      load_frags(wf, xf, kt & 1, 0);
      if constexpr (decltype(next1)::value) dma_w(sw);
      bar();
      mfma32(wf, xf, No{}, 0, first);
      bar();
      load_w(wf, kt & 1, 1);
      bar();
      mfma32(wf, xf, next2, sa, No{});
      if constexpr (decltype(next2)::value)
        asm volatile("s_waitcnt vmcnt(4)" ::: "memory");
      else
        asm volatile("s_waitcnt vmcnt(0)" ::: "memory");
      return;
    }
    if constexpr (SP) {
      bar();
      load_frags(wf, xf, kt & 1, 0);
      bar();
      mfma32(wf, xf, No{}, 0, first);
      bar();
      load_w(wfl, kt & 1, 1);
      if constexpr (decltype(next1)::value) dma_w(sw);
      bar();
      mfma32(wfl, xf, No{}, 0, No{});
      bar();
      load_x(xf, kt & 1, 1);
      bar();
      mfma32(wf, xf, next2, sa, No{});
      if constexpr (decltype(next2)::value)
        asm volatile("s_waitcnt vmcnt(4)" ::: "memory");
      else
        asm volatile("s_waitcnt vmcnt(0)" ::: "memory");
      return;
    }
    bar();
    load_frags(wf, xf, kt & 1, 0);
    if constexpr (decltype(next1)::value) dma_w(sw);
    bar();
    mfma32(wf, xf, No{}, 0, first);
    bar();
    load_frags(wf, xf, kt & 1, 1);
    bar();
    mfma32(wf, xf, next2, sa, No{});
    if constexpr (decltype(next2)::value)
      asm volatile("s_waitcnt vmcnt(4)" ::: "memory");
    else
      asm volatile("s_waitcnt vmcnt(0)" ::: "memory");
  };
  auto stage1 = [&](int kt, auto next1, auto next2, int sw, int sa, auto first) {
    if constexpr (SP && SP2) {
      bar();
      load_frags(wf, xf, kt & 1, 0);
      if constexpr (decltype(next1)::value) dma_w(sw);
      bar();
      mfma32(wf, xf, No{}, 0, first);
      bar();
      load_w(wf, kt & 1, 1);
      asm volatile("s_waitcnt vmcnt(0)" ::: "memory");
      bar();
      mfma32(wf, xf, next2, sa, No{});
      return;
    }
    if constexpr (SP) {
      bar();
      load_frags(wf, xf, kt & 1, 0);
      bar();
      mfma32(wf, xf, No{}, 0, first);
      bar();
      load_w(wfl, kt & 1, 1);
      if constexpr (decltype(next1)::value) dma_w(sw);
      bar();
      mfma32(wfl, xf, No{}, 0, No{});
      bar();
      load_x(xf, kt & 1, 1);
      asm volatile("s_waitcnt vmcnt(0)" ::: "memory");
      bar();
      mfma32(wf, xf, next2, sa, No{});
      return;
    }
    bar();
    load_frags(wf, xf, kt & 1, 0);
    if constexpr (decltype(next1)::value) dma_w(sw);
    bar();
    mfma32(wf, xf, No{}, 0, first);
    bar();
    load_frags(wf, xf, kt & 1, 1);
    asm volatile("s_waitcnt vmcnt(0)" ::: "memory");
    bar();
    mfma32(wf, xf, next2, sa, No{});
  };

  const bool ln = KIND == 1 && p.ln_stats != nullptr;
#if defined(MK_LN_ABL) && MK_LN_ABL == 1
  const bool ln_fast = false && ln;
#define MK_LN_NO_SLOW 1
#else
  const bool ln_fast = ln && p.ln_nslot == 16;
#endif
  LnRowLoads16 lnl;
  if (ln_fast) lnl.issue(p, m0, tid);
  constexpr bool PRODUCER = AMODE == A_DENSE && (KIND == 2 || KIND == 3);
  ShiftLoad shl;
  if constexpr (PRODUCER) shl.issue(p, m0, tid, 256);
  dma_a(0);
  dma_w(0);
  if constexpr (!PERSIST) dma_a(1);
  constexpr int YOUNGER = PERSIST ? 8 : 12;
  const bool publish = ln && p.ln_shift_out != nullptr && n0 == 0;
  if (ln_fast) lnl.template finish<YOUNGER>(p, tid, (float2*)(smem + 2 * STAGE_BYTES), m0, publish);
#ifndef MK_LN_NO_SLOW
  else if (ln) ln_params_to_lds<256, 512>(p, m0, tid, (float2*)(smem + 2 * STAGE_BYTES), publish);
#endif
  if constexpr (PRODUCER) shl.template finish<YOUNGER>(tid, 256, (float*)(smem + 2 * STAGE_BYTES));
  if constexpr (!PERSIST) asm volatile("s_waitcnt vmcnt(4)" ::: "memory");
  const int bstep = PERSIST ? (int)gridDim.x : 0;
  for (;;) {
    const int nbid = bid + bstep;
    const bool has_next = PERSIST && nbid < ntiles;
    int m1 = m0, n1 = n0;
    if (PERSIST && has_next) tile_origin(nbid, m1, n1);
    if constexpr (PERSIST) {
      refresh_lane();
      derive_lane();
      set_aoff(m0);
      set_woff(n0);
      dma_a(1);
      if (bid == (int)blockIdx.x) asm volatile("s_waitcnt vmcnt(4)" ::: "memory");
    }
    bool ln_pending = false;
    auto first_stage_done = [&]() {
      if constexpr (PERSIST) {
        if (ln_pending) {
          const bool publish1 = ln && p.ln_shift_out != nullptr && n0 == 0;
          if (ln_fast) {
            LnRowDma16::finish<0>(p, wave, lane, (float2*)(smem + 2 * STAGE_BYTES), smem + LN_STAGE_OFF, m0, publish1);
            asm volatile("s_waitcnt lgkmcnt(0)" ::: "memory");
            LnRowDma16::issue<2>(p, m0, wave, lane, smem + LN_STAGE_OFF);
          }
          if constexpr (PRODUCER) shl.template finish<-1>(tid, 256, (float*)(smem + 2 * STAGE_BYTES));
        }
      }
    };
    auto second_stage_done = [&]() {
      if constexpr (PERSIST) {
        if (ln_pending && ln_fast)
          LnRowDma16::finish<2>(p, wave, lane, (float2*)(smem + 2 * STAGE_BYTES), smem + LN_STAGE_OFF, m0,
                                ln && p.ln_shift_out != nullptr && n0 == 0);
      }
    };
    ln_pending = PERSIST && bid != (int)blockIdx.x;
    int kt0 = 0;
    if (wm == 0) {
      if constexpr (PERSIST) {
        stage0(0, Yes{}, Yes{}, 1, 2, Yes{});
        first_stage_done();
        stage0(1, Yes{}, Yes{}, 2, 3, No{});
        second_stage_done();
        kt0 = 2;
      }
      for (int kt = kt0; kt < nk - 2; ++kt) stage0(kt, Yes{}, Yes{}, kt + 1, kt + 2, No{});
      if constexpr (PERSIST) {
        set_aoff(m1);
        stage0(nk - 2, Yes{}, Yes{}, nk - 1, 0, No{});
        set_woff(n1);
        stage0(nk - 1, Yes{}, No{}, 0, 0, No{});
      } else {
        stage0(nk - 2, Yes{}, No{}, nk - 1, 0, No{});
        stage0(nk - 1, No{}, No{}, 0, 0, No{});
      }
      bar();
    } else {
      bar();
      if constexpr (PERSIST) {
        stage1(0, Yes{}, Yes{}, 1, 2, Yes{});
        first_stage_done();
        stage1(1, Yes{}, Yes{}, 2, 3, No{});
        second_stage_done();
        kt0 = 2;
      }
      for (int kt = kt0; kt < nk - 2; ++kt) stage1(kt, Yes{}, Yes{}, kt + 1, kt + 2, No{});
      if constexpr (PERSIST) {
        set_aoff(m1);
        stage1(nk - 2, Yes{}, Yes{}, nk - 1, 0, No{});
        set_woff(n1);
        stage1(nk - 1, Yes{}, No{}, 0, 0, No{});
      } else {
        stage1(nk - 2, Yes{}, No{}, nk - 1, 0, No{});
        stage1(nk - 1, No{}, No{}, 0, 0, No{});
      }
    }
    char* wl0 = smem + STAGE_BYTES + wave * 4096;
    refresh_lane();
    epilogue_lds<T, KIND, AMODE == A_CONV3>(p, acc, wl0, wl0 + A_BYTES, m0, n0, wm, wn, lane, g, (const float2*)(smem + 2 * STAGE_BYTES));
    if (!(PERSIST && has_next)) break;
    bid = nbid;
    m0 = m1;
    n0 = n1;
    asm volatile("" : "+s"(m0), "+s"(n0));
    refresh_lane();
    if (ln_fast) LnRowDma16::issue<0>(p, m0, wave, lane, smem + LN_STAGE_OFF);
    if constexpr (PRODUCER) shl.issue(p, m0, tid, 256);
  }
}

template <typename T, int AMODE, int KIND, bool PERSIST, bool SP = false, bool SP2 = false>
int launch_k2(const GemmParams& p, int groups, hipStream_t st, int band_m, int grid) {
  constexpr int LDS = 2 * 512 * 128 + 256 * 8 + (PERSIST && KIND == 1 ? 16384 : 0);
  static bool attr_done = false;
  if (!attr_done) {
    hipError_t e = hipFuncSetAttribute((const void*)gemm_pp64_kernel<T, AMODE, KIND, PERSIST, SP, SP2>, hipFuncAttributeMaxDynamicSharedMemorySize, LDS);
    if (e != hipSuccess) {
      mk_set_error("gemm: cannot reserve %d B of LDS: %s", LDS, hipGetErrorString(e));
      return MK_ERR_LAUNCH;
    }
    attr_done = true;
  }
  hipLaunchKernelGGL((gemm_pp64_kernel<T, AMODE, KIND, PERSIST, SP, SP2>), dim3(grid, groups, 1), dim3(512), LDS, st, p, band_m);
  MK_CHECK_LAUNCH();
  return MK_OK;
}

template <typename T, int AMODE, int KIND>
int launch_k(const GemmParams& p, int groups, hipStream_t st, int band_m) {
  const int ntm = (p.M + 255) / 256, ntn = (p.N + 255) / 256;
  if (band_m == 0) band_m = (AMODE == A_DENSE && ntn <= 4) ? -4 : 8;
  if constexpr (KIND == 0 && sizeof(T) == 2 && std::is_same<T, _Float16>::value) {
    if (p.npass == 2) {
      if constexpr (AMODE == A_CONV3) return launch_k2<T, AMODE, 0, false, true, true>(p, groups, st, band_m, ntm * ntn);
    }
    if (p.npass > 1) return launch_k2<T, AMODE, 0, false, true>(p, groups, st, band_m, ntm * ntn);
  }
  if constexpr (AMODE == A_DENSE && KIND != 0) {
    const int nk = p.K / BK, grid = num_cus() & ~7;
    const bool ok = groups == 1 && p.npass <= 1 && (nk & 1) == 0 && nk >= 4 && grid >= 8 && ntm * ntn > grid &&
                    !(KIND == 1 && p.ln_stats && p.ln_nslot != 16);
    if (g_pp64_persist != 1 && ok && !(g_pp64_persist == 2 && KIND == 1)) return launch_k2<T, AMODE, KIND, true>(p, groups, st, band_m, grid);
  }
  return launch_k2<T, AMODE, KIND, false>(p, groups, st, band_m, ntm * ntn);
}

template <typename T>
int launch_dense(const GemmParams& p, int groups, hipStream_t st, int band_m) {
  if (p.xh && p.epi == MK_EPI_LS_RESIDUAL && p.out_f32) return launch_k<T, A_DENSE, 3>(p, groups, st, band_m);
  if (p.xh) return launch_k<T, A_DENSE, 2>(p, groups, st, band_m);
  if (p.ln_stats) return launch_k<T, A_DENSE, 1>(p, groups, st, band_m);
  return launch_k<T, A_DENSE, 0>(p, groups, st, band_m);
}

}

int launch_pp64(const GemmParams& p, int groups, int dtype, int amode, hipStream_t st, int band_m) {
  if (amode == A_DENSE) return dtype == MK_BF16 ? launch_dense<__bf16>(p, groups, st, band_m) : launch_dense<_Float16>(p, groups, st, band_m);
  return dtype == MK_BF16 ? launch_k<__bf16, A_CONV3, 0>(p, groups, st, band_m) : launch_k<_Float16, A_CONV3, 0>(p, groups, st, band_m);
}

}
}
```

### mickey_amd/ops.py

```python

import numpy as np
import torch


from ._native import ACT_GELU, ACT_NONE, ACT_RELU, call, dtype_code, ptr, query, stream

LOG2E = 1.4426950408889634


def _chk(t, dtype=None):
    assert t.is_cuda and t.is_contiguous(), "expected a contiguous device tensor"
    if dtype is not None:
        assert t.dtype == dtype, "expected %s, got %s" % (dtype, t.dtype)
    return t


def preprocess_u8(frames, H, W, out=None):
    assert frames.is_cuda and frames.dtype == torch.uint8 and frames.dim() == 4 and frames.shape[3] == 3 and frames.is_contiguous()
    n, Hs, Ws, _ = frames.shape
    if out is None:
        out = torch.empty((n, 3, H, W), device=frames.device, dtype=torch.float32)
    call("mk_preprocess_u8", ptr(frames), Hs * Ws * 3, n, Hs, Ws, ptr(out), H, W, stream())
    return out


def gemm_set_tile(mode):
    call("mk_gemm_set_tile", int(mode))


def gemm(a, w, bias=None, act=ACT_NONE, out_f32=False, out=None, lda=None, K=None):
    M = a.shape[0]
    lda = a.shape[1] if lda is None else lda
    N, ldw = w.shape
    K = min(lda, ldw) if K is None else K
    if out is None:
        out = torch.empty((M, N), device=a.device, dtype=torch.float32 if out_f32 else a.dtype)
    call("mk_gemm", ptr(a), lda, ptr(w), ldw, ptr(bias), ptr(out), out.stride(0), M, N, K, act,
         int(out.dtype == torch.float32), dtype_code(a.dtype), stream())
    return out


def gemm_grouped(a, w, bias, out, groups, M, N, K, lda, ldw, ldc, stride_a, stride_w, stride_bias, stride_out, act=ACT_NONE):
    call("mk_gemm_grouped", ptr(a), lda, stride_a, ptr(w), ldw, stride_w, ptr(bias), stride_bias, ptr(out), ldc, stride_out,
         groups, M, N, K, act, int(out.dtype == torch.float32), dtype_code(a.dtype), stream())
    return out


def gemm_ls_residual(a, w, bias, gamma, x):
    M, K = a.shape
    N = w.shape[0]
    call("mk_gemm_ls_residual", ptr(a), a.stride(0), ptr(w), w.stride(0), ptr(bias), ptr(gamma), ptr(x), x.stride(0), M, N, K,
         dtype_code(a.dtype), stream())
    return x


def gemm_qkv(a, w, bias, q, k, vt, nimg, ntok, ntok_pad, heads):
    qscale = (64.0 ** -0.5) * LOG2E
    call("mk_gemm_qkv", ptr(a), a.stride(0), ptr(w), w.stride(0), ptr(bias), ptr(q), ptr(k), ptr(vt), nimg, ntok, ntok_pad,
         heads, qscale, dtype_code(a.dtype), stream())


def gemm_ls_residual_ln(a, w, bias, gamma, xh, xl, stats, x_out=None, shift=None):
    M, K = a.shape
    N = w.shape[0]
    call("mk_gemm_ls_residual_ln", ptr(a), a.stride(0), ptr(w), w.stride(0), ptr(bias), ptr(gamma), ptr(xh), ptr(xl),
         xh.stride(0), ptr(stats), ptr(shift), ptr(x_out), x_out.stride(0) if x_out is not None else N, M, N, K,
         dtype_code(a.dtype), stream())


def gemm_patch_embed_ln(a, w, bias, pos, xh, xl, stats, nimg, npatch):
    D = w.shape[0]
    call("mk_gemm_patch_embed_ln", ptr(a), a.stride(0), ptr(w), w.stride(0), ptr(bias), ptr(pos), ptr(xh), ptr(xl), ptr(stats),
         nimg, npatch, D, w.shape[1], dtype_code(a.dtype), stream())


def cls_token_ln(cls, pos, xh, xl, stats, nimg, ntok, D):
    call("mk_cls_token_ln", ptr(cls), ptr(pos), ptr(xh), ptr(xl), ptr(stats), nimg, ntok, D, dtype_code(xh.dtype), stream())


def recentre_split(xh, xl, stats):
    rows, D = xh.shape
    call("mk_recentre_split", ptr(xh), ptr(xl), ptr(stats), rows, D, dtype_code(xh.dtype), stream())


def gemm_ln(a, w, bias, colsum, stats, eps, act=ACT_NONE, out=None, shift_out=None):
    M, K = a.shape
    N = w.shape[0]
    if out is None:
        out = torch.empty((M, N), device=a.device, dtype=a.dtype)
    call("mk_gemm_ln", ptr(a), a.stride(0), ptr(w), w.stride(0), ptr(bias), ptr(colsum), ptr(stats), float(eps), ptr(shift_out),
         ptr(out), out.stride(0), M, N, K, act, dtype_code(a.dtype), stream())
    return out


def gemm_qkv_ln(a, w, bias, colsum, stats, eps, q, k, vt, nimg, ntok, ntok_pad, heads, shift_out=None):
    qscale = (64.0 ** -0.5) * LOG2E
    call("mk_gemm_qkv_ln", ptr(a), a.stride(0), ptr(w), w.stride(0), ptr(bias), ptr(colsum), ptr(stats), float(eps),
         ptr(shift_out), ptr(q), ptr(k), ptr(vt), nimg, ntok, ntok_pad, heads, qscale, dtype_code(a.dtype), stream())


def im2col_patch14(img, gh, gw, ldo, dtype, out=None):
    assert img.dtype == torch.float32 and img.stride(3) == 1
    nimg = img.shape[0]
    if out is None:
        out = torch.empty((nimg * gh * gw, ldo), device=img.device, dtype=dtype)
    assert out.shape == (nimg * gh * gw, ldo) and out.dtype == dtype and out.is_contiguous()
    call("mk_im2col_patch14", ptr(img), img.stride(0), img.stride(1), img.stride(2), nimg, gh, gw, ptr(out), ldo,
         dtype_code(dtype), stream())
    return out


def gemm_patch_embed(a, w, bias, pos, x, nimg, npatch):
    D = w.shape[0]
    call("mk_gemm_patch_embed", ptr(a), a.stride(0), ptr(w), w.stride(0), ptr(bias), ptr(pos), ptr(x), nimg, npatch, D,
         w.shape[1], dtype_code(a.dtype), stream())


def cls_token(cls, pos, x, nimg, ntok, D):
    call("mk_cls_token", ptr(cls), ptr(pos), ptr(x), nimg, ntok, D, stream())


def layernorm(x, w, b, eps, out=None, out_dtype=torch.bfloat16, resid=None, rows_out=None, rows_per_img=None, skip=0,
              ldo=None, wgroup_rows=0, ldx=None, ldr=None, bordered=None, sat=None):
    D = w.shape[-1]
    rows_in = x.numel() // x.shape[-1]
    if rows_per_img is None:
        rows_per_img = rows_in
    if rows_out is None:
        rows_out = rows_in - skip * (rows_in // rows_per_img)
    if isinstance(out, (tuple, list)):
        oh, ol = out
        assert oh.dtype == torch.float16 and (ol is None or (ol.dtype == torch.float16 and oh.stride() == ol.stride()))
        ldo = oh.stride(-2) if ldo is None else ldo
        bh, bw, bm = (bordered[1], bordered[2], bordered[0] * bordered[1] * bordered[2]) if bordered else (0, 0, 0)
        call("mk_layernorm_planes", ptr(x), x.stride(-2) if ldx is None else ldx, ptr(w), ptr(b), float(eps), ptr(oh), ptr(ol), ldo,
             SPLIT_ACT_SCALE, ptr(resid), (resid.stride(-2) if resid is not None else D) if ldr is None else ldr, rows_out, D,
             rows_per_img, skip, wgroup_rows, bh, bw, bm, sat_word(sat), stream())
        return out
    if out is None and out_dtype is not None:
        out = torch.empty((rows_out, D), device=x.device, dtype=out_dtype)
    is_f32 = out is not None and out.dtype == torch.float32
    ldo = (out.stride(-2) if out is not None else D) if ldo is None else ldo
    lp = out.dtype if (out is not None and not is_f32) else torch.bfloat16
    bh, bw, bm = (bordered[1], bordered[2], bordered[0] * bordered[1] * bordered[2]) if bordered else (0, 0, 0)
    call("mk_layernorm", ptr(x), x.stride(-2) if ldx is None else ldx, ptr(w), ptr(b), float(eps), ptr(out), ldo, int(is_f32),
         ptr(resid), (resid.stride(-2) if resid is not None else D) if ldr is None else ldr, rows_out, D, rows_per_img, skip,
         wgroup_rows, bh, bw, bm, dtype_code(lp), stream())
    return out


def gemm_ln128(a, w, ln_w, ln_b, eps, out, groups, M, K, lda=None, ldo=None, resid=None, bordered=None):
    assert a.dtype == w.dtype == out.dtype and w.shape[-2] == 128 and w.shape[-1] == K
    lda = a.stride(-2) if lda is None else lda
    ldo = out.stride(-2) if ldo is None else ldo
    bh, bw = (bordered[1], bordered[2]) if bordered else (0, 0)
    call("mk_gemm_ln128", ptr(a), lda, a.stride(0) if a.dim() == 3 else 0, ptr(w), w.stride(-2), w.stride(0) if w.dim() == 3 else 0, ptr(ln_w), ptr(ln_b),
         float(eps), ptr(resid), resid.stride(-2) if resid is not None else 128, ptr(out), ldo, groups, M, K, bh, bw, dtype_code(a.dtype),
         stream())
    return out


def attn_set_mode(mode):
    call("mk_attn_set_mode", int(mode))


def flash_attn(q, k, vt, out, nimg, heads, ntok, ntok_pad):
    call("mk_flash_attn_fwd", ptr(q), ptr(k), ptr(vt), ptr(out), out.stride(0), nimg, heads, ntok, ntok_pad,
         dtype_code(q.dtype), stream())
    return out


CONV_OUT_DENSE, CONV_OUT_BORDERED, CONV_OUT_F32 = 0, 1, 2


def bordered_rows(nimg, H, W):
    return int(query("mk_bordered_rows", nimg, H, W))


def bordered_empty(lead, nimg, H, W, C, dtype, device):
    return torch.zeros(tuple(lead) + (bordered_rows(nimg, H, W), C), dtype=dtype, device=device)


def bordered_index(nimg, H, W, device):
    b, y, x = torch.meshgrid(torch.arange(nimg, device=device), torch.arange(H, device=device),
                             torch.arange(W, device=device), indexing="ij")
    return (((b * (H + 1) + y + 1) * (W + 1)) + x + 1).reshape(-1)


def conv3x3(in1, C1, w, bias, out, Cout, groups, nimg, H, W, act=ACT_NONE, in2=None, C2=0, resid=None,
            stride_in1=0, stride_in2=0, stride_w=0, stride_bias=0, stride_out=0, stride_resid=0, out_bordered=False):
    kind = CONV_OUT_F32 if out.dtype == torch.float32 and in1.dtype != torch.float32 else \
        (CONV_OUT_BORDERED if out_bordered else CONV_OUT_DENSE)
    call("mk_conv3x3", ptr(in1), stride_in1, C1, ptr(in2), stride_in2, C2, ptr(w), w.shape[-1], stride_w, ptr(bias), stride_bias,
         ptr(resid), stride_resid, ptr(out), Cout, stride_out, groups, nimg, H, W, act, kind, dtype_code(in1.dtype), stream())
    return out


SPLIT_ACT_SCALE, SPLIT_W_SCALE = 64.0, 1024.0


def sat_word(flag):
    if flag is None:
        return None
    assert flag.dtype == torch.int32 and flag.numel() >= 1 and flag.is_cuda
    return ptr(flag)


def plane_pair(shape, device, zero=False):
    t = (torch.zeros if zero else torch.empty)((2,) + tuple(shape), device=device, dtype=torch.float16)
    return t[0], t[1]


def split_planes(x, hi, lo, scale=SPLIT_ACT_SCALE, sat=None):
    assert x.dtype == torch.float32 and hi.dtype == torch.float16 and lo.dtype == torch.float16 and hi.shape == x.shape == lo.shape
    cols = x.shape[-1]
    rows = x.numel() // cols

    def ld(t):
        assert t.stride(-1) == 1
        lead = t.stride(-2) if t.dim() > 1 else cols
        for d in range(t.dim() - 2):
            assert t.stride(d) == t.stride(d + 1) * t.shape[d + 1], "rows must be equidistant"
        return lead
    assert ld(hi) == ld(lo)
    call("mk_split_planes", ptr(x), rows, cols, ld(x), float(scale), ptr(hi), ptr(lo), ld(hi), sat_word(sat), stream())
    return hi, lo


def gemm_grouped_split(a, w, bias, out, groups, M, N, K, lda, ldc, stride_a, stride_w, stride_bias, stride_out, act=ACT_NONE,
                       w_scale=SPLIT_W_SCALE, sat=None):
    ah, al = a
    assert w.dtype == torch.float16 and w.shape[-1] == 2 * K
    if isinstance(out, (tuple, list)):
        oh, ol = out
    else:
        oh, ol = out, None
        assert out.dtype == torch.float32
    call("mk_gemm_grouped_split", ptr(ah), ptr(al), lda, stride_a, ptr(w), 2 * K, stride_w, ptr(bias), stride_bias, ptr(oh), ptr(ol),
         ldc, stride_out, groups, M, N, K, act, 1.0 / (SPLIT_ACT_SCALE * float(w_scale)), SPLIT_ACT_SCALE, sat_word(sat), stream())
    return out


def conv3x3_split(in1, C1, w, bias, out, Cout, groups, nimg, H, W, act=ACT_NONE, in2=None, C2=0, stride_in1=0, stride_in2=0,
                  stride_w=0, stride_bias=0, stride_out=0, out_bordered=False, w_scale=SPLIT_W_SCALE, sat=None):
    assert w.dtype == torch.float16
    h1, l1 = in1
    h2, l2 = in2 if in2 is not None else (None, None)
    if isinstance(out, (tuple, list)):
        oh, ol = out
        assert oh.dtype == torch.float16 and ol.dtype == torch.float16 and oh.shape == ol.shape
    else:
        oh, ol = out, None
        assert out.dtype == torch.float32
    call("mk_conv3x3_split", ptr(h1), ptr(l1), stride_in1, C1, ptr(h2), ptr(l2), stride_in2, C2, ptr(w), w.shape[-1], stride_w,
         ptr(bias), stride_bias, ptr(oh), ptr(ol), Cout, stride_out, groups, nimg, H, W, act, int(out_bordered),
         1.0 / (SPLIT_ACT_SCALE * float(w_scale)), SPLIT_ACT_SCALE, sat_word(sat), stream())
    return out


def posenc_add(x, pe, xs, cat, groups, nimg, npix, C):
    call("mk_posenc_add", ptr(x), ptr(pe), ptr(xs), ptr(cat), cat.stride(-2), groups, nimg, npix, C, dtype_code(x.dtype),
         stream())


def linattn_work_floats(groups, nimg, L, C):
    return query("mk_linattn_work_floats", groups, nimg, L, C)


def linattn_kv(qkv, kv, work, groups, nimg, L, C):
    call("mk_linattn_kv", ptr(qkv), ptr(kv), ptr(work), groups, nimg, L, C, stream())


def linattn_apply(qkv, kv, out, ldo, groups, nimg, L, C):
    call("mk_linattn_apply", ptr(qkv), ptr(kv), ptr(out), ldo, groups, nimg, L, C, dtype_code(out.dtype), stream())


def head_tails(f_det, w_score, f_off, w_xy, f_dep, w_dep, f_dsc, nimg, h, w, C, Cd, border=3, use_softmax=True,
               use_depth_sigmoid=False, max_depth=60.0, norm_dsc=True, down=14.0):
    dev = f_det.device
    n = h * w
    scr = torch.empty((nimg, 1, n), device=dev, dtype=torch.float32)
    kps = torch.empty((nimg, 2, n), device=dev, dtype=torch.float32)
    depth = torch.empty((nimg, 1, n), device=dev, dtype=torch.float32)
    dsc = torch.empty((nimg, Cd, n), device=dev, dtype=torch.float32)
    call("mk_head_tails", ptr(f_det), ptr(w_score), ptr(f_off), ptr(w_xy), ptr(f_dep), ptr(w_dep), ptr(f_dsc), ptr(scr),
         ptr(kps), ptr(depth), ptr(dsc), nimg, h, w, C, Cd, border, int(use_softmax), int(use_depth_sigmoid), float(max_depth),
         int(norm_dsc), float(down), stream())
    return scr, kps, depth, dsc


def dual_softmax_split_ok(C, temperature):
    return C == 128 and temperature > 0 and LOG2E / float(temperature) <= 100.0


def check_keyframe_index(index, B, K):
    if torch.is_tensor(index):
        if index.dtype.is_floating_point or index.dtype.is_complex or index.dtype == torch.bool:
            raise ValueError("keyframe_index must hold integers, got %s" % index.dtype)
        a = index.detach().cpu().numpy()
    else:
        a = np.asarray(index)
        if a.size == 0 and a.dtype == np.float64:
            a = a.astype(np.int64)
        if a.dtype.kind not in "iu":
            raise ValueError("keyframe_index must hold integers, got %s" % a.dtype)
    if a.ndim != 1 or a.shape[0] != int(B):
        raise ValueError("keyframe_index must hold one entry per pair (%d), got shape %s" % (int(B), tuple(a.shape)))
    if not 0 < int(K) <= max(1, int(B)):
        raise ValueError("keyframe mode needs 1 <= K <= B keyframes (image0 has %d for %d pairs: a keyframe no pair uses is "
                         "wasted work)" % (int(K), int(B)))
    if a.size and (int(a.min()) < 0 or int(a.max()) >= int(K)):
        raise ValueError("keyframe_index entries must lie in [0, %d), got [%d, %d]" % (int(K), int(a.min()), int(a.max())))
    return a.astype(np.int32)


def _kf_arg(keyframe_index, B, K, dev):
    if keyframe_index is None:
        return None, B
    t = keyframe_index
    if not (torch.is_tensor(t) and t.is_cuda and t.dtype == torch.int32 and t.is_contiguous() and t.dim() == 1 and t.shape[0] == B):
        t = torch.from_numpy(check_keyframe_index(t, B, K)).to(dev)
    return t, K


def dual_softmax(dsc0, dsc1, scr0=None, scr1=None, temperature=0.1, dustbin=None, want_scores=True, want_kp=True,
                 want_final=True, split=False, keyframe_index=None):
    _chk(dsc0, torch.float32)
    _chk(dsc1, torch.float32)
    K, C, n0 = dsc0.shape
    B, n1 = dsc1.shape[0], dsc1.shape[2]
    if keyframe_index is None:
        assert K == B, "dsc0 and dsc1 hold different batch counts (keyframe mode needs keyframe_index)"
    dev = dsc0.device
    kf, kfn = _kf_arg(keyframe_index, B, K, dev)
    mk = lambda want: torch.empty((B, n0, n1), device=dev, dtype=torch.float32) if want else None
    scores = mk(want_scores)
    kp = mk(want_kp and scr0 is not None)
    fin = mk(want_final and scr0 is not None)
    if split:
        work = torch.empty((query("mk_dual_softmax_split_work_floats", B, n0, n1),), device=dev, dtype=torch.float32)
        args = (ptr(dsc0), ptr(dsc1), ptr(scr0), ptr(scr1), 1.0 / float(temperature), int(dustbin is not None),
                float(dustbin) if dustbin is not None else 0.0, ptr(scores), ptr(kp), ptr(fin), ptr(work), B, C, n0, n1)
        if kf is None:
            call("mk_dual_softmax_split", *args, stream())
        else:
            call("mk_dual_softmax_split_kf", *args, ptr(kf), kfn, stream())
        return scores, kp, fin
    work = torch.empty((query("mk_dual_softmax_work_floats", B, n0, n1, int(scores is None and fin is None)),), device=dev,
                       dtype=torch.float32)
    args = (ptr(dsc0), ptr(dsc1), ptr(scr0), ptr(scr1), 1.0 / float(temperature), int(dustbin is not None),
            float(dustbin) if dustbin is not None else 0.0, ptr(scores), ptr(kp), ptr(fin), ptr(work), B, C, n0, n1)
    if kf is None:
        call("mk_dual_softmax", *args, stream())
    else:
        call("mk_dual_softmax_kf", *args, ptr(kf), kfn, stream())
    return scores, kp, fin


def dual_softmax_train_fwd(dsc0, dsc1, scr0, scr1, temperature, dustbin, split):
    B, C, n0 = dsc0.shape
    n1 = dsc1.shape[2]
    dev = dsc0.device
    out = torch.empty((B, n0, n1), device=dev, dtype=torch.float32)
    lse = torch.empty((B, 2, max(n0, n1)), device=dev, dtype=torch.float32)
    work = torch.empty((query("mk_dual_softmax_train_work_floats", B, n0, n1, int(split)),), device=dev, dtype=torch.float32)
    has_kp = scr0 is not None
    call("mk_dual_softmax_train", ptr(dsc0), ptr(dsc1), ptr(scr0), ptr(scr1), 1.0 / float(temperature), ptr(dustbin),
         None if has_kp else ptr(out), None, ptr(out) if has_kp else None, ptr(lse), ptr(work), B, C, n0, n1, int(split), stream())
    return out, lse


def dual_softmax_bwd(dsc0, dsc1, scr0, scr1, temperature, dustbin, lse, G, split, need):
    B, C, n0 = dsc0.shape
    n1 = dsc1.shape[2]
    dev = dsc0.device
    shapes = ((B, C, n0), (B, C, n1), (B, n0), (B, n1), (B,))
    outs = [torch.empty(sh, device=dev, dtype=torch.float32) if want else None for sh, want in zip(shapes, need)]
    work = torch.empty((query("mk_dual_softmax_bwd_work_floats", B, n0, n1, int(split)),), device=dev, dtype=torch.float32)
    call("mk_dual_softmax_bwd", ptr(dsc0), ptr(dsc1), ptr(scr0), ptr(scr1), 1.0 / float(temperature), ptr(dustbin), ptr(lse),
         ptr(G), *[ptr(o) for o in outs], ptr(work), B, C, n0, n1, int(split), stream())
    return tuple(outs)


def sinkhorn(dsc0, dsc1, alpha, iters=10, scr0=None, scr1=None, want_scores=True, want_kp=False, want_final=False,
             keyframe_index=None):
    K, C, n0 = dsc0.shape
    B, n1 = dsc1.shape[0], dsc1.shape[2]
    if keyframe_index is None:
        assert K == B, "dsc0 and dsc1 hold different batch counts (keyframe mode needs keyframe_index)"
    dev = dsc0.device
    kf, kfn = _kf_arg(keyframe_index, B, K, dev)
    mk = lambda want: torch.empty((B, n0, n1), device=dev, dtype=torch.float32) if want else None
    out, kp, fin = mk(want_scores), mk(want_kp and scr0 is not None), mk(want_final and scr0 is not None)
    work = torch.empty((query("mk_sinkhorn_work_floats", B, n0, n1),), device=dev, dtype=torch.float32)
    args = (ptr(dsc0), ptr(dsc1), ptr(scr0), ptr(scr1), float(alpha), int(iters), ptr(out), ptr(kp), ptr(fin), ptr(work), B, C, n0, n1)
    if kf is None:
        call("mk_sinkhorn", *args, stream())
    else:
        call("mk_sinkhorn_kf", *args, ptr(kf), kfn, stream())
    return out if scr0 is None else (out, kp, fin)


def mutual_nn(scores):
    _chk(scores, torch.float32)
    B, n0, n1 = scores.shape
    dev = scores.device
    matches = torch.zeros((B, n0, 2), device=dev, dtype=torch.int32)
    count = torch.zeros((B,), device=dev, dtype=torch.int32)
    work = torch.empty((2 * B * (n0 + n1),), device=dev, dtype=torch.int32)
    call("mk_mutual_nn", ptr(scores), ptr(matches), ptr(count), ptr(work), B, n0, n1, stream())
    return matches, count



def counter_add(counter, inc):
    call("mk_counter_add", ptr(counter), int(inc), stream())


def dev_mfma_sustained(device, iters=400000, zero_operands=False, workgroups=None):
    wg = workgroups or torch.cuda.get_device_properties(device).multi_processor_count
    scratch = torch.empty((wg * 512,), device=device, dtype=torch.float32)
    call("mk_dev_mfma_sustained", ptr(scratch), wg, max(1, iters // 8), int(zero_operands), stream())
    e0, e1 = torch.cuda.Event(enable_timing=True), torch.cuda.Event(enable_timing=True)
    e0.record()
    call("mk_dev_mfma_sustained", ptr(scratch), wg, iters, int(zero_operands), stream())
    e1.record()
    e1.synchronize()
    return wg * iters * 1048576.0 / (e0.elapsed_time(e1) * 1e-3) / 1e12


def exprace_work(B, rows_per_pair, k, ncell, device):
    work = torch.empty((query("mk_exprace_topk_work_bytes", B, rows_per_pair, k, ncell),), device=device, dtype=torch.uint8)
    work[:query("mk_exprace_topk_state_bytes", B, rows_per_pair)].zero_()
    return work


def exprace_topk(p, rows_per_pair, k, noise=None, seed=0, offset=0, invalid=None, offset_dev=None, pair_base=0, work=None):
    p, noise = _c(p, noise)
    _chk(p, torch.float32)
    B, ncell = p.shape
    dev = p.device
    idx = torch.empty((B * rows_per_pair, k), device=dev, dtype=torch.int32)
    cnt = torch.empty((B * rows_per_pair,), device=dev, dtype=torch.int32)
    if work is None:
        work = exprace_work(B, rows_per_pair, k, ncell, dev)
    assert work.numel() >= query("mk_exprace_topk_work_bytes", B, rows_per_pair, k, ncell)
    try:
        call("mk_exprace_topk", ptr(p), ptr(noise), int(seed), int(offset), ptr(offset_dev), ptr(idx), ptr(cnt), ptr(invalid),
             ptr(work), B, rows_per_pair, ncell, k, int(pair_base), stream())
    except Exception:
        work[:query("mk_exprace_topk_state_bytes", B, rows_per_pair)].zero_()
        raise
    return idx, cnt


def _c(*ts):
    return [None if t is None else t.contiguous() for t in ts]


def gather_backproject(idx, final_scores, kps0, depth0, kps1, depth1, K0, K1, rows_per_pair, keyframe_index=None):
    idx, final_scores, kps0, depth0, kps1, depth1, K0, K1 = _c(idx, final_scores, kps0, depth0, kps1, depth1, K0, K1)
    B, n0, n1 = final_scores.shape
    R, k = idx.shape
    dev = idx.device
    kf, kfn = _kf_arg(keyframe_index, B, kps0.shape[0], dev)
    X = torch.empty((R, k, 3), device=dev, dtype=torch.float32)
    Y = torch.empty((R, k, 3), device=dev, dtype=torch.float32)
    wts = torch.empty((R, k), device=dev, dtype=torch.float32)
    corr = torch.empty((R, k, 6), device=dev, dtype=torch.float32)
    args = (ptr(idx), ptr(final_scores), ptr(kps0), ptr(depth0), ptr(kps1), ptr(depth1), ptr(K0), ptr(K1), ptr(X), ptr(Y),
            ptr(wts), ptr(corr), B, rows_per_pair, k, n0, n1)
    if kf is None:
        call("mk_gather_backproject", *args, stream())
    else:
        call("mk_gather_backproject_kf", *args, ptr(kf), kfn, stream())
    return X, Y, wts, corr


def ransac_hypotheses(X, Y, wts, it_ransac, th_soft, noise3=None, idx3_in=None, seed=0, offset=0, offset_dev=None, set_base=0):
    X, Y, wts, noise3, idx3_in = _c(X, Y, wts, noise3, idx3_in)
    nsets, k, _ = X.shape
    dev = X.device
    nh = nsets * it_ransac
    Rh = torch.empty((nh, 9), device=dev, dtype=torch.float32)
    th = torch.empty((nh, 3), device=dev, dtype=torch.float32)
    score = torch.empty((nh,), device=dev, dtype=torch.float32)
    idx3 = torch.empty((nh, 3), device=dev, dtype=torch.int32)
    call("mk_ransac_hypotheses", ptr(X), ptr(Y), ptr(wts), ptr(noise3), ptr(idx3_in), int(seed), int(offset), ptr(offset_dev),
         float(th_soft), ptr(Rh), ptr(th), ptr(score), ptr(idx3), nsets, it_ransac, k, int(set_base), stream())
    return Rh, th, score, idx3


def train_ransac_masks(X, Y, wts, it_ransac, th_ref, num_ref, num_corr, noise=None, idx_in=None, seed=0, offset=0,
                       offset_dev=None, set_base=0):
    X, Y, wts, noise, idx_in = _c(X, Y, wts, noise, idx_in)
    _chk(X, torch.float32)
    nsets, S, _ = X.shape
    dev = X.device
    nh = nsets * it_ransac
    if idx_in is not None:
        idx_in = idx_in.to(torch.int32)
    mask = torch.empty((nh, S), device=dev, dtype=torch.float32)
    idx = torch.empty((nh, num_corr), device=dev, dtype=torch.int32)
    rounds = torch.empty((nh,), device=dev, dtype=torch.int32)
    call("mk_train_ransac_masks", ptr(X), ptr(Y), ptr(wts), ptr(noise), ptr(idx_in), int(seed), int(offset), ptr(offset_dev),
         float(th_ref), int(num_ref), int(num_corr), ptr(mask), ptr(idx), ptr(rounds), nsets, it_ransac, S, int(set_base),
         stream())
    return mask, idx, rounds


def reinforce_scatter(idx, loss_value, B, it_matches, ncell):
    idx, loss_value = _c(idx.to(torch.int32), loss_value.to(torch.float32))
    S = idx.shape[1]
    dev = idx.device
    grads = torch.zeros((B, ncell), device=dev, dtype=torch.float32)
    grads_b = torch.zeros((B, ncell), device=dev, dtype=torch.float32)
    call("mk_reinforce_scatter", ptr(idx), ptr(loss_value), ptr(grads), ptr(grads_b), B, it_matches, S, ncell, stream())
    return grads, grads_b

def train_tail_fwd(X, Y, mask, Rgt, tgt, K0, K1, it_ransac, it_matches, th_soft, loss_type, soft_clip, img_h=720.0):
    X, Y, mask, Rgt, tgt, K0, K1 = _c(X, Y, mask, Rgt, tgt, K0, K1)
    nsets, S, _ = X.shape
    nh = nsets * it_ransac
    dev = X.device
    out = torch.empty((nh, 4), device=dev, dtype=torch.float32)
    Rt = torch.empty((nh, 12), device=dev, dtype=torch.float32)
    saved = torch.zeros((nh, 32), device=dev, dtype=torch.float32)
    call("mk_train_tail_fwd", ptr(X), ptr(Y), ptr(mask), ptr(Rgt), ptr(tgt), ptr(K0), ptr(K1), nsets, it_ransac, S, it_matches,
         float(th_soft), int(loss_type), int(soft_clip), float(img_h), ptr(out), ptr(Rt), ptr(saved), stream())
    return out, Rt, saved


def train_tail_bwd(X, Y, mask, Rgt, tgt, K0, K1, it_ransac, it_matches, th_soft, loss_type, soft_clip, Rt, saved, grad_out,
                   img_h=720.0):
    X, Y, mask, Rgt, tgt, K0, K1, grad_out = _c(X, Y, mask, Rgt, tgt, K0, K1, grad_out)
    nsets, S, _ = X.shape
    dev = X.device
    work = torch.empty((nsets * it_ransac, 16), device=dev, dtype=torch.float32)
    gX, gY = torch.empty_like(X), torch.empty_like(Y)
    call("mk_train_tail_bwd", ptr(X), ptr(Y), ptr(mask), ptr(Rgt), ptr(tgt), ptr(K0), ptr(K1), nsets, it_ransac, S, it_matches,
         float(th_soft), int(loss_type), int(soft_clip), float(img_h), ptr(Rt), ptr(saved), ptr(grad_out), ptr(work), ptr(gX),
         ptr(gY), stream())
    return gX, gY


def train_aggregate_fwd(out, Rt, saved, B, it_matches, it_ransac, temperature, add_null, null_loss, null_score):
    out, Rt, saved = _c(out, Rt, saved)
    dev = out.device
    loss_value = torch.empty((B * it_matches,), device=dev, dtype=torch.float32)
    per_pair = torch.empty((B, 3), device=dev, dtype=torch.float32)
    coef = torch.empty((B * it_matches * it_ransac, 2), device=dev, dtype=torch.float32)
    flags = torch.zeros((2,), device=dev, dtype=torch.int32)
    call("mk_train_aggregate_fwd", ptr(out), ptr(Rt), ptr(saved), B, it_matches, it_ransac, float(temperature), int(bool(add_null)),
         float(null_loss), float(null_score), ptr(loss_value), ptr(per_pair), ptr(coef), ptr(flags), stream())
    return loss_value, per_pair, coef, flags


def train_aggregate_bwd(coef, g_pair, B, it_matches, it_ransac):
    coef, g_pair = _c(coef, g_pair.float())
    g = torch.empty_like(coef)
    call("mk_train_aggregate_bwd", ptr(coef), ptr(g_pair), B, it_matches, it_ransac, ptr(g), stream())
    return g


def gather_backproject_bwd(idx, corr, gX, gY, K0, K1, B, rows_per_pair, n0, n1):
    idx, corr, gX, gY, K0, K1 = _c(idx, corr, gX, gY, K0, K1)
    k = idx.shape[1]
    buf = torch.zeros((B * 3 * (n0 + n1),), device=idx.device, dtype=torch.float32)
    gk0, gd0 = buf[:2 * B * n0].view(B, 2, n0), buf[2 * B * n0:3 * B * n0].view(B, 1, n0)
    o = 3 * B * n0
    gk1, gd1 = buf[o:o + 2 * B * n1].view(B, 2, n1), buf[o + 2 * B * n1:].view(B, 1, n1)
    call("mk_gather_backproject_bwd", ptr(idx), ptr(corr), ptr(gX), ptr(gY), ptr(K0), ptr(K1), ptr(gk0), ptr(gd0), ptr(gk1), ptr(gd1),
         B, rows_per_pair, k, n0, n1, stream())
    return gk0, gd0, gk1, gd1


def refine_pose(X, Y, Rh, th, score, B, it_matches, it_ransac, th_inlier, num_ref, min_inliers, invalid=None):
    X, Y, Rh, th, score = _c(X, Y, Rh, th, score)
    k = X.shape[1]
    dev = X.device
    R = torch.empty((B, 3, 3), device=dev, dtype=torch.float32)
    t = torch.empty((B, 1, 3), device=dev, dtype=torch.float32)
    conf = torch.empty((B, 1), device=dev, dtype=torch.float32)
    best = torch.empty((B,), device=dev, dtype=torch.int32)
    mask = torch.empty((B, k), device=dev, dtype=torch.uint8)
    rounds = torch.empty((B,), device=dev, dtype=torch.int32)
    if invalid is None:
        invalid = torch.zeros((1,), device=dev, dtype=torch.int32)
    call("mk_refine_pose", ptr(X), ptr(Y), ptr(Rh), ptr(th), ptr(score), float(th_inlier), int(num_ref), int(min_inliers),
         ptr(R), ptr(t), ptr(conf), ptr(best), ptr(mask), ptr(rounds), ptr(invalid), B, it_matches, it_ransac, k, stream())
    call("mk_pose_finalize", ptr(R), ptr(t), ptr(conf), ptr(invalid), B, stream())
    return R, t, conf, best, mask, rounds, invalid
```

Measured before the change: 266.0.

## Add short-row tail tiles for persistent pp64 GEMM wave quantization

Result: no change. 266.2 (median of 6 runs) (+0.1%).

```diff
diff --git a/include/mickey_hip_dev.h b/include/mickey_hip_dev.h
--- a/include/mickey_hip_dev.h
+++ b/include/mickey_hip_dev.h
@@ -7,6 +7,8 @@
 
 int mk_gemm_set_tile(int mode);
 
+int mk_dev_gemm_tail_plan(int M, int N, int cus, int* out3);
+
 int mk_attn_set_mode(int mode);
 
 int mk_dev_mfma_sustained(float* scratch, int workgroups, int iters, int zero_operands, void* stream);
diff --git a/mickey_amd/_native.py b/mickey_amd/_native.py
--- a/mickey_amd/_native.py
+++ b/mickey_amd/_native.py
@@ -76,6 +76,7 @@
 
 DEV_SIGNATURES = {
     "mk_gemm_set_tile": ("i", "i"),
+    "mk_dev_gemm_tail_plan": ("i", "iiip"),
     "mk_attn_set_mode": ("i", "i"),
     "mk_dev_mfma_sustained": ("i", "piiip"),
 }
diff --git a/mickey_amd/csrc/mk_gemm.hip b/mickey_amd/csrc/mk_gemm.hip
--- a/mickey_amd/csrc/mk_gemm.hip
+++ b/mickey_amd/csrc/mk_gemm.hip
@@ -175,6 +175,15 @@
 
 extern "C" {
 
+int mk_dev_gemm_tail_plan(int M, int N, int cus, int* out3) {
+  MK_CHECK_ARG(out3 != nullptr, "mk_dev_gemm_tail_plan: null output");
+  const TailPlan t = plan_tail(M, N, cus & ~7);
+  out3[0] = t.body_rows;
+  out3[1] = t.tail_bm;
+  out3[2] = t.tail_tiles;
+  return MK_OK;
+}
+
 int mk_gemm_set_tile(int mode) {
   if (mode >= 400 && mode < 464) {
     g_band_m = mode - 400;
@@ -190,6 +199,10 @@
   }
   if (mode >= 600 && mode <= 602) {
     g_pp64_persist = mode - 600;
+    return MK_OK;
+  }
+  if (mode == 610 || mode == 611) {
+    g_pp64_tail = mode == 610;
     return MK_OK;
   }
   MK_CHECK_ARG(mode == 0 || mode == 1 || mode == 2 || mode == 7,
diff --git a/mickey_amd/csrc/mk_gemm_common.hpp b/mickey_amd/csrc/mk_gemm_common.hpp
--- a/mickey_amd/csrc/mk_gemm_common.hpp
+++ b/mickey_amd/csrc/mk_gemm_common.hpp
@@ -155,10 +155,10 @@
 
 struct ShiftLoad {
   float v;
-  __device__ __forceinline__ void issue(const GemmParams& p, int m0, int tid, int BM) {
+  __device__ __forceinline__ void issue(const GemmParams& p, int m0, int tid, int BM, int rph = 128) {
     v = 0.f;
     if (p.ln_shift_in && tid < BM) {
-      int m = m0 + tid;
+      int m = rph == 128 ? m0 + tid : m0 + (tid >> 7) * rph + (tid & 127);
       m = m < p.M ? m : p.M - 1;
       const float* a = p.ln_shift_in + m;
       asm volatile("global_load_dword %0, %1, off" : "=v"(v) : "v"(a) : "memory");
@@ -514,15 +514,16 @@
   }
 }
 
-template <typename T, int EPI, int ACT, bool HAS_BIAS, bool LN = false, bool SPLIT = false, bool FIN = false, bool CONV = false>
-__device__ __forceinline__ void epilogue_lds_impl(const GemmParams& p, f32x4 (&acc)[8][4], char* wl0, char* wl1, int m0, int n0, int wm,
+template <typename T, int EPI, int ACT, bool HAS_BIAS, bool LN = false, bool SPLIT = false, bool FIN = false, bool CONV = false, int WMF = 8>
+__device__ __forceinline__ void epilogue_lds_impl(const GemmParams& p, f32x4 (&acc)[WMF][4], char* wl0, char* wl1, int m0, int n0, int wm,
                                                   int wn, int lane, int g, const float2* lnp = nullptr) {
+  static_assert(WMF == 8 || (SPLIT && (WMF == 6 || WMF == 4 || WMF == 2)), "short-row tiles: the split-stream epilogues only");
   using V4 = typename Lp<T>::V4;
   using V8 = typename Lp<T>::V8;
   const int fr = lane & 15, fg = lane >> 4;
   const float* bias = HAS_BIAS ? p.bias + (long long)g * p.strideBias_g : nullptr;
   const int nw = n0 + wn * 64;
-  const int mw = m0 + wm * 128;
+  const int mw = m0 + wm * (WMF * 16);
   int img0 = 0, tok0 = 0;
   if (EPI == MK_EPI_QKV) {
     img0 = mw / p.ntok;
@@ -551,7 +552,7 @@
 #pragma unroll
   for (int mi = 0; mi < 8; ++mi) prm[mi] = LN ? lnp[wm * 128 + mi * 16 + fr] : make_float2(1.f, 0.f);
   const bool lp_out = EPI == MK_EPI_QKV || (EPI == MK_EPI_STORE && !p.out_f32 && !p.out_lo);
-  if (lp_out) {
+  if (WMF == 8 && lp_out) {
     int which = 0, head = 0;
     if (EPI == MK_EPI_QKV) {
       const int D = p.heads * 64;
@@ -803,7 +804,20 @@
         }
       }
     };
-    if (SPLIT && !FIN && EPI == MK_EPI_LS_RESIDUAL) {
+    if constexpr (WMF < 8) {
+      preload(0, 0, WMF >= 4 ? 16 : 8);
+      stageq(0, 0);
+      drain(0, 0, 8);
+      if (WMF == 6) preload(1, 0, 8);
+      if (WMF >= 4) {
+        stageq(0, 1);
+        drain(0, 8, 16);
+      }
+      if (WMF == 6) {
+        stageq(1, 0);
+        drain(1, 0, 8);
+      }
+    } else if (SPLIT && !FIN && EPI == MK_EPI_LS_RESIDUAL) {
       preload(0, 0, 16);
       stageq(0, 0);
       drain(0, 0, 8);
@@ -830,20 +844,21 @@
   }
 }
 
-template <typename T, int KIND, bool CONV = false, int BN = 256>
-__device__ __forceinline__ void epilogue_lds(const GemmParams& p, f32x4 (&acc)[8][4], char* wl0, char* wl1, int m0, int n0, int wm,
+template <typename T, int KIND, bool CONV = false, int BN = 256, int WMF = 8>
+__device__ __forceinline__ void epilogue_lds(const GemmParams& p, f32x4 (&acc)[WMF][4], char* wl0, char* wl1, int m0, int n0, int wm,
                                              int wn, int lane, int g, const float2* lnp = nullptr) {
+  static_assert(WMF == 8 || KIND == 2 || KIND == 3, "short-row tiles: producers only");
   if constexpr (KIND == 2 || KIND == 3) {
-    const bool interior = m0 + 256 <= p.M && n0 + BN <= p.N;
+    const bool interior = m0 + 32 * WMF <= p.M && n0 + BN <= p.N;
     if (KIND == 3) {
-      if (interior) epilogue_lds_impl<T, MK_EPI_LS_RESIDUAL, MK_ACT_NONE, true, false, true, true>(p, acc, wl0, wl1, m0, n0, wm, wn, lane, g, lnp);
-      else epilogue_impl<T, 8, MK_EPI_LS_RESIDUAL, MK_ACT_NONE, true, false, true>(p, acc, m0, n0, wm, wn, lane, g);
+      if (interior) epilogue_lds_impl<T, MK_EPI_LS_RESIDUAL, MK_ACT_NONE, true, false, true, true, false, WMF>(p, acc, wl0, wl1, m0, n0, wm, wn, lane, g, lnp);
+      else epilogue_impl<T, WMF, MK_EPI_LS_RESIDUAL, MK_ACT_NONE, true, false, true>(p, acc, m0, n0, wm, wn, lane, g);
     } else if (p.epi == MK_EPI_PATCH) {
-      if (interior) epilogue_lds_impl<T, MK_EPI_PATCH, MK_ACT_NONE, true, false, true>(p, acc, wl0, wl1, m0, n0, wm, wn, lane, g);
-      else epilogue_impl<T, 8, MK_EPI_PATCH, MK_ACT_NONE, true, false, true>(p, acc, m0, n0, wm, wn, lane, g);
+      if (interior) epilogue_lds_impl<T, MK_EPI_PATCH, MK_ACT_NONE, true, false, true, false, false, WMF>(p, acc, wl0, wl1, m0, n0, wm, wn, lane, g);
+      else epilogue_impl<T, WMF, MK_EPI_PATCH, MK_ACT_NONE, true, false, true>(p, acc, m0, n0, wm, wn, lane, g);
     } else {
-      if (interior) epilogue_lds_impl<T, MK_EPI_LS_RESIDUAL, MK_ACT_NONE, true, false, true, false>(p, acc, wl0, wl1, m0, n0, wm, wn, lane, g, lnp);
-      else epilogue_impl<T, 8, MK_EPI_LS_RESIDUAL, MK_ACT_NONE, true, false, true>(p, acc, m0, n0, wm, wn, lane, g);
+      if (interior) epilogue_lds_impl<T, MK_EPI_LS_RESIDUAL, MK_ACT_NONE, true, false, true, false, false, WMF>(p, acc, wl0, wl1, m0, n0, wm, wn, lane, g, lnp);
+      else epilogue_impl<T, WMF, MK_EPI_LS_RESIDUAL, MK_ACT_NONE, true, false, true>(p, acc, m0, n0, wm, wn, lane, g);
     }
   } else if constexpr (KIND == 1) {
 #if defined(MK_LN_ABL) && MK_LN_ABL == 2
@@ -892,6 +907,13 @@
 
 int num_cus();
 extern int g_pp64_persist;
+extern int g_pp64_tail;
+struct TailPlan {
+  int body_rows;
+  int tail_bm;
+  int tail_tiles;
+};
+TailPlan plan_tail(int M, int N, int grid);
 int launch_pp64(const GemmParams& p, int groups, int dtype, int amode, hipStream_t st, int band_m);
 int launch_f32(const GemmParams& p, int groups, int amode, hipStream_t st);
 
diff --git a/mickey_amd/csrc/mk_gemm_pp64.hip b/mickey_amd/csrc/mk_gemm_pp64.hip
--- a/mickey_amd/csrc/mk_gemm_pp64.hip
+++ b/mickey_amd/csrc/mk_gemm_pp64.hip
@@ -5,380 +5,41 @@
 namespace mk {
 namespace gemm {
 int g_pp64_persist = 2;
+int g_pp64_tail = 1;
+
+TailPlan plan_tail(int M, int N, int grid) {
+  TailPlan t{M, 0, 0};
+  if (M <= 0 || N <= 0 || grid <= 0) return t;
+  const long long ntn = (N + 255) / 256, ntm = (M + 255) / 256;
+  const long long tiles = ntm * ntn, rounds = tiles / grid;
+  if (rounds < 2 || tiles % grid == 0) return t;
+  const long long body_m = rounds * grid / ntn;
+  if (body_m * ntn <= grid) return t;
+  const long long rows = (long long)M - body_m * 256;
+  for (int bm = 192; bm >= 64; bm -= 64) {
+    const long long tt = (rows + bm - 1) / bm * ntn;
+    if (tt <= grid) {
+      t.body_rows = (int)(body_m * 256);
+      t.tail_bm = bm;
+      t.tail_tiles = (int)tt;
+      return t;
+    }
+  }
+  return t;
+}
 namespace {
 
 template <typename T, int AMODE, int KIND, bool PERSIST = false, bool SP = false, bool SP2 = false>
 __global__ __launch_bounds__(512, 2) void gemm_pp64_kernel(GemmParams p, int band_m) {
-  static_assert(!SP2 || SP, "SP2 is a form of the split-operand kernel");
-  static_assert(!PERSIST || AMODE == A_DENSE, "the persistent tile loop is built for dense operands");
-  static_assert(!SP || (KIND == 0 && !PERSIST && sizeof(T) == 2), "split operands: plain epilogues, one tile per workgroup");
-  constexpr int BKA = SP ? BK / 2 : BK;
-  using V8 = typename Lp<T>::V8;
-  constexpr int WMF = 8, BM = 256, BN = 256;
-  constexpr int A_BYTES = BM * 128, STAGE_BYTES = (BM + BN) * 128;
-  constexpr int LN_STAGE_OFF = 2 * STAGE_BYTES + 256 * 8;
-  extern __shared__ __attribute__((aligned(16))) char smem[];
+  constexpr int WMF = 8;
+#include "mk_gemm_pp64_body.hpp"
+}
 
-  const int tid0 = threadIdx.x;
-  const int wave = __builtin_amdgcn_readfirstlane(tid0 >> 6);
-  int lane = tid0 & 63, tid = tid0;
-  auto refresh_lane = [&]() {
-    if constexpr (PERSIST) {
-      asm volatile("v_mbcnt_lo_u32_b32 %0, -1, 0\n\tv_mbcnt_hi_u32_b32 %0, -1, %0" : "=v"(lane));
-      tid = wave * 64 + lane;
-    }
-  };
-  const int wm = wave >> 2, wn = wave & 3;
-  const int g = blockIdx.y;
-  const int ntm = (p.M + BM - 1) / BM, ntn = (p.N + BN - 1) / BN;
-  const int nk = p.K / BK;
-
-  const T* A = (const T*)p.A + (long long)g * p.strideA_g;
-  const T* A2 = p.A2 ? (const T*)p.A2 + (long long)g * p.strideA2_g : nullptr;
-  const T* W = (const T*)p.W + (long long)g * p.strideW_g;
-  int srow = lane >> 3, sp = lane & 7;
-  const int ntiles = ntm * ntn;
-  auto tile_origin = [&](int id, int& mm, int& nn) {
-    int tm, tn;
-    pp_tile_coords(xcd_remap(id, ntiles), ntm, ntn, band_m, tm, tn);
-    mm = tm * BM;
-    nn = tn * BN;
-  };
-  int bid = blockIdx.x;
-  int m0, n0;
-  tile_origin(bid, m0, n0);
-  unsigned woff[4], aoff[4], aoff2[4];
-  auto set_woff = [&](int nn0) {
-#pragma unroll
-    for (int j = 0; j < 4; ++j) {
-      const int rw = (wave * 4 + j) * 8 + srow;
-      int n = nn0 + rw;
-      n = n < p.N ? n : p.N - 1;
-      woff[j] = ((unsigned)n * (unsigned)p.ldw + swz8(rw, sp) * 8) * (unsigned)sizeof(T);
-    }
-  };
-  auto set_aoff = [&](int mm0) {
-#pragma unroll
-    for (int j = 0; j < 4; ++j) {
-      const int ra = wm * 128 + (wn * 4 + j) * 8 + srow;
-      int m = mm0 + ra;
-      m = m < p.M ? m : p.M - 1;
-      const int c = swz8(ra, sp);
-      const unsigned cc = SP ? (unsigned)(c & 3) : (unsigned)c;
-      const bool lo = SP && (c >> 2) != 0;
-      const unsigned pb1 = !SP ? 0u : (lo ? p.pl1[1] : p.pl1[0]), pb2 = !SP ? 0u : (lo ? p.pl2[1] : p.pl2[0]);
-      if (AMODE == A_DENSE) {
-        aoff[j] = ((unsigned)m * (unsigned)p.lda + cc * 8) * (unsigned)sizeof(T) + pb1;
-        aoff2[j] = 0;
-      } else {
-        const unsigned br = (unsigned)bordered_row(m, p.H, p.Wd);
-        aoff[j] = (br * (unsigned)p.C1 + cc * 8) * (unsigned)sizeof(T) + pb1;
-        aoff2[j] = (br * (unsigned)p.C2 + cc * 8) * (unsigned)sizeof(T) + pb2;
-      }
-    }
-  };
-  set_woff(n0);
-  set_aoff(m0);
-  auto dma_w1 = [&](int s, int j) {
-    glds16_sv(W + s * BK, woff[j], smem + (s & 1) * STAGE_BYTES + A_BYTES + (wave * 4 + j) * 1024);
-  };
-  const int ntap = A2 ? 10 : 9;
-  const T* cbase = AMODE == A_DENSE ? A : A - (long long)(p.Wd + 2) * p.C1;
-  int cleft = p.C1, ctap = 0;
-  auto conv_advance = [&]() {
-    cleft -= BKA;
-    const bool wrap = cleft == 0;
-    ctap += wrap ? 1 : 0;
-    const int ty = (ctap * 11) >> 5, tx = ctap - 3 * ty;
-    const T* tapbase = ctap < 9 ? A + (long long)((ty - 1) * (p.Wd + 1) + tx - 1) * p.C1 : A2;
-    cbase = wrap ? tapbase : cbase + BKA;
-    cleft = wrap ? (ctap < 9 ? p.C1 : p.C2) : cleft;
-  };
-  auto dma_a1 = [&](int s, int j) {
-    char* dst = smem + (s & 1) * STAGE_BYTES + (wm * 16 + wn * 4 + j) * 1024;
-    if (AMODE == A_DENSE) {
-      glds16_sv(A + s * BKA, aoff[j], dst);
-    } else {
-      glds16_sv(cbase, ctap < 9 ? aoff[j] : aoff2[j], dst);
-    }
-  };
-  auto dma_w = [&](int s) {
-#pragma unroll
-    for (int j = 0; j < 4; ++j) dma_w1(s, j);
-  };
-  auto dma_a = [&](int s) {
-#pragma unroll
-    for (int j = 0; j < 4; ++j) dma_a1(s, j);
-    if (AMODE != A_DENSE) conv_advance();
-  };
-
-  int fr = lane & 15, fg = lane >> 4;
-  auto derive_lane = [&]() {
-    srow = lane >> 3;
-    sp = lane & 7;
-    fr = lane & 15;
-    fg = lane >> 4;
-  };
-  auto load_w = [&](V8* wf, int par, int h) {
-    const char* sW = smem + par * STAGE_BYTES + A_BYTES;
-#pragma unroll
-    for (int i = 0; i < 4; ++i) {
-      const int rw = wn * 64 + i * 16 + fr;
-      wf[i] = *(const V8*)(sW + rw * 128 + swz8(rw, h * 4 + fg) * 16);
-    }
-  };
-  auto load_x = [&](V8* xf, int par, int h) {
-    const char* sA = smem + par * STAGE_BYTES;
-#pragma unroll
-    for (int i = 0; i < WMF; ++i) {
-      const int rx = wm * 128 + i * 16 + fr;
-      xf[i] = *(const V8*)(sA + rx * 128 + swz8(rx, h * 4 + fg) * 16);
-    }
-  };
-  auto load_frags = [&](V8* wf, V8* xf, int par, int h) {
-    load_w(wf, par, h);
-    load_x(xf, par, h);
-  };
-  f32x4 acc[WMF][4];
-  auto zero_acc = [&]() {
-#pragma unroll
-    for (int i = 0; i < WMF; ++i)
-#pragma unroll
-      for (int j = 0; j < 4; ++j) acc[i][j] = f32x4{0.f, 0.f, 0.f, 0.f};
-  };
-  if constexpr (!PERSIST) zero_acc();
-  auto mfma32 = [&](const V8* wf, const V8* xf, auto dma, int s, auto first) {
-    constexpr bool DMA = decltype(dma)::value;
-    constexpr bool FIRST = decltype(first)::value;
-    __builtin_amdgcn_s_setprio(1);
-    __builtin_amdgcn_sched_barrier(0);
-#pragma unroll
-    for (int q = 0; q < 32; ++q) {
-      const int mi = q >> 2, ni = q & 3;
-      acc[mi][ni] = Lp<T>::mma16(wf[ni], xf[mi], FIRST ? f32x4{0.f, 0.f, 0.f, 0.f} : acc[mi][ni]);
-      if (DMA && (q & 7) == 3) {
-        __builtin_amdgcn_sched_barrier(0);
-        dma_a1(s, q >> 3);
-        __builtin_amdgcn_sched_barrier(0);
-      }
-    }
-    __builtin_amdgcn_sched_barrier(0);
-    __builtin_amdgcn_s_setprio(0);
-    if (DMA && AMODE != A_DENSE) conv_advance();
-  };
-  auto bar = [&]() {
-    asm volatile("s_waitcnt lgkmcnt(0)" ::: "memory");
-    __builtin_amdgcn_s_barrier();
-  };
-  using Yes = std::integral_constant<bool, true>;
-  using No = std::integral_constant<bool, false>;
-  V8 wf[4], xf[WMF];
-  V8 wfl[SP ? 4 : 1];
-  auto stage0 = [&](int kt, auto next1, auto next2, int sw, int sa, auto first) {
-    if constexpr (SP && SP2) {
-      bar();
-      load_frags(wf, xf, kt & 1, 0);
-      if constexpr (decltype(next1)::value) dma_w(sw);
-      bar();
-      mfma32(wf, xf, No{}, 0, first);
-      bar();
-      load_w(wf, kt & 1, 1);
-      bar();
-      mfma32(wf, xf, next2, sa, No{});
-      if constexpr (decltype(next2)::value)
-        asm volatile("s_waitcnt vmcnt(4)" ::: "memory");
-      else
-        asm volatile("s_waitcnt vmcnt(0)" ::: "memory");
-      return;
-    }
-    if constexpr (SP) {
-      bar();
-      load_frags(wf, xf, kt & 1, 0);
-      bar();
-      mfma32(wf, xf, No{}, 0, first);
-      bar();
-      load_w(wfl, kt & 1, 1);
-      if constexpr (decltype(next1)::value) dma_w(sw);
-      bar();
-      mfma32(wfl, xf, No{}, 0, No{});
-      bar();
-      load_x(xf, kt & 1, 1);
-      bar();
-      mfma32(wf, xf, next2, sa, No{});
-      if constexpr (decltype(next2)::value)
-        asm volatile("s_waitcnt vmcnt(4)" ::: "memory");
-      else
-        asm volatile("s_waitcnt vmcnt(0)" ::: "memory");
-      return;
-    }
-    bar();
-    load_frags(wf, xf, kt & 1, 0);
-    if constexpr (decltype(next1)::value) dma_w(sw);
-    bar();
-    mfma32(wf, xf, No{}, 0, first);
-    bar();
-    load_frags(wf, xf, kt & 1, 1);
-    bar();
-    mfma32(wf, xf, next2, sa, No{});
-    if constexpr (decltype(next2)::value)
-      asm volatile("s_waitcnt vmcnt(4)" ::: "memory");
-    else
-      asm volatile("s_waitcnt vmcnt(0)" ::: "memory");
-  };
-  auto stage1 = [&](int kt, auto next1, auto next2, int sw, int sa, auto first) {
-    if constexpr (SP && SP2) {
-      bar();
-      load_frags(wf, xf, kt & 1, 0);
-      if constexpr (decltype(next1)::value) dma_w(sw);
-      bar();
-      mfma32(wf, xf, No{}, 0, first);
-      bar();
-      load_w(wf, kt & 1, 1);
-      asm volatile("s_waitcnt vmcnt(0)" ::: "memory");
-      bar();
-      mfma32(wf, xf, next2, sa, No{});
-      return;
-    }
-    if constexpr (SP) {
-      bar();
-      load_frags(wf, xf, kt & 1, 0);
-      bar();
-      mfma32(wf, xf, No{}, 0, first);
-      bar();
-      load_w(wfl, kt & 1, 1);
-      if constexpr (decltype(next1)::value) dma_w(sw);
-      bar();
-      mfma32(wfl, xf, No{}, 0, No{});
-      bar();
-      load_x(xf, kt & 1, 1);
-      asm volatile("s_waitcnt vmcnt(0)" ::: "memory");
-      bar();
-      mfma32(wf, xf, next2, sa, No{});
-      return;
-    }
-    bar();
-    load_frags(wf, xf, kt & 1, 0);
-    if constexpr (decltype(next1)::value) dma_w(sw);
-    bar();
-    mfma32(wf, xf, No{}, 0, first);
-    bar();
-    load_frags(wf, xf, kt & 1, 1);
-    asm volatile("s_waitcnt vmcnt(0)" ::: "memory");
-    bar();
-    mfma32(wf, xf, next2, sa, No{});
-  };
-
-  const bool ln = KIND == 1 && p.ln_stats != nullptr;
-#if defined(MK_LN_ABL) && MK_LN_ABL == 1
-  const bool ln_fast = false && ln;
-#define MK_LN_NO_SLOW 1
-#else
-  const bool ln_fast = ln && p.ln_nslot == 16;
-#endif
-  LnRowLoads16 lnl;
-  if (ln_fast) lnl.issue(p, m0, tid);
-  constexpr bool PRODUCER = AMODE == A_DENSE && (KIND == 2 || KIND == 3);
-  ShiftLoad shl;
-  if constexpr (PRODUCER) shl.issue(p, m0, tid, 256);
-  dma_a(0);
-  dma_w(0);
-  if constexpr (!PERSIST) dma_a(1);
-  constexpr int YOUNGER = PERSIST ? 8 : 12;
-  const bool publish = ln && p.ln_shift_out != nullptr && n0 == 0;
-  if (ln_fast) lnl.template finish<YOUNGER>(p, tid, (float2*)(smem + 2 * STAGE_BYTES), m0, publish);
-#ifndef MK_LN_NO_SLOW
-  else if (ln) ln_params_to_lds<256, 512>(p, m0, tid, (float2*)(smem + 2 * STAGE_BYTES), publish);
-#endif
-  if constexpr (PRODUCER) shl.template finish<YOUNGER>(tid, 256, (float*)(smem + 2 * STAGE_BYTES));
-  if constexpr (!PERSIST) asm volatile("s_waitcnt vmcnt(4)" ::: "memory");
-  const int bstep = PERSIST ? (int)gridDim.x : 0;
-  for (;;) {
-    const int nbid = bid + bstep;
-    const bool has_next = PERSIST && nbid < ntiles;
-    int m1 = m0, n1 = n0;
-    if (PERSIST && has_next) tile_origin(nbid, m1, n1);
-    if constexpr (PERSIST) {
-      refresh_lane();
-      derive_lane();
-      set_aoff(m0);
-      set_woff(n0);
-      dma_a(1);
-      if (bid == (int)blockIdx.x) asm volatile("s_waitcnt vmcnt(4)" ::: "memory");
-    }
-    bool ln_pending = false;
-    auto first_stage_done = [&]() {
-      if constexpr (PERSIST) {
-        if (ln_pending) {
-          const bool publish1 = ln && p.ln_shift_out != nullptr && n0 == 0;
-          if (ln_fast) {
-            LnRowDma16::finish<0>(p, wave, lane, (float2*)(smem + 2 * STAGE_BYTES), smem + LN_STAGE_OFF, m0, publish1);
-            asm volatile("s_waitcnt lgkmcnt(0)" ::: "memory");
-            LnRowDma16::issue<2>(p, m0, wave, lane, smem + LN_STAGE_OFF);
-          }
-          if constexpr (PRODUCER) shl.template finish<-1>(tid, 256, (float*)(smem + 2 * STAGE_BYTES));
-        }
-      }
-    };
-    auto second_stage_done = [&]() {
-      if constexpr (PERSIST) {
-        if (ln_pending && ln_fast)
-          LnRowDma16::finish<2>(p, wave, lane, (float2*)(smem + 2 * STAGE_BYTES), smem + LN_STAGE_OFF, m0,
-                                ln && p.ln_shift_out != nullptr && n0 == 0);
-      }
-    };
-    ln_pending = PERSIST && bid != (int)blockIdx.x;
-    int kt0 = 0;
-    if (wm == 0) {
-      if constexpr (PERSIST) {
-        stage0(0, Yes{}, Yes{}, 1, 2, Yes{});
-        first_stage_done();
-        stage0(1, Yes{}, Yes{}, 2, 3, No{});
-        second_stage_done();
-        kt0 = 2;
-      }
-      for (int kt = kt0; kt < nk - 2; ++kt) stage0(kt, Yes{}, Yes{}, kt + 1, kt + 2, No{});
-      if constexpr (PERSIST) {
-        set_aoff(m1);
-        stage0(nk - 2, Yes{}, Yes{}, nk - 1, 0, No{});
-        set_woff(n1);
-        stage0(nk - 1, Yes{}, No{}, 0, 0, No{});
-      } else {
-        stage0(nk - 2, Yes{}, No{}, nk - 1, 0, No{});
-        stage0(nk - 1, No{}, No{}, 0, 0, No{});
-      }
-      bar();
-    } else {
-      bar();
-      if constexpr (PERSIST) {
-        stage1(0, Yes{}, Yes{}, 1, 2, Yes{});
-        first_stage_done();
-        stage1(1, Yes{}, Yes{}, 2, 3, No{});
-        second_stage_done();
-        kt0 = 2;
-      }
-      for (int kt = kt0; kt < nk - 2; ++kt) stage1(kt, Yes{}, Yes{}, kt + 1, kt + 2, No{});
-      if constexpr (PERSIST) {
-        set_aoff(m1);
-        stage1(nk - 2, Yes{}, Yes{}, nk - 1, 0, No{});
-        set_woff(n1);
-        stage1(nk - 1, Yes{}, No{}, 0, 0, No{});
-      } else {
-        stage1(nk - 2, Yes{}, No{}, nk - 1, 0, No{});
-        stage1(nk - 1, No{}, No{}, 0, 0, No{});
-      }
-    }
-    char* wl0 = smem + STAGE_BYTES + wave * 4096;
-    refresh_lane();
-    epilogue_lds<T, KIND, AMODE == A_CONV3>(p, acc, wl0, wl0 + A_BYTES, m0, n0, wm, wn, lane, g, (const float2*)(smem + 2 * STAGE_BYTES));
-    if (!(PERSIST && has_next)) break;
-    bid = nbid;
-    m0 = m1;
-    n0 = n1;
-    asm volatile("" : "+s"(m0), "+s"(n0));
-    refresh_lane();
-    if (ln_fast) LnRowDma16::issue<0>(p, m0, wave, lane, smem + LN_STAGE_OFF);
-    if constexpr (PRODUCER) shl.issue(p, m0, tid, 256);
-  }
+template <typename T, int KIND, int WMF>
+__global__ __launch_bounds__(512, 2) void gemm_pp_tail_kernel(GemmParams p, int band_m) {
+  constexpr int AMODE = A_DENSE;
+  constexpr bool PERSIST = false, SP = false, SP2 = false;
+#include "mk_gemm_pp64_body.hpp"
 }
 
 template <typename T, int AMODE, int KIND, bool PERSIST, bool SP = false, bool SP2 = false>
@@ -398,6 +59,33 @@
   return MK_OK;
 }
 
+template <typename T, int KIND>
+int launch_tail(const GemmParams& p0, int body_rows, hipStream_t st, int band_m) {
+  constexpr int LDS = 2 * 512 * 128 + 256 * 8;
+  static bool attr_done = false;
+  if (!attr_done) {
+    hipError_t e = hipFuncSetAttribute((const void*)gemm_pp_tail_kernel<T, KIND, 6>, hipFuncAttributeMaxDynamicSharedMemorySize, LDS);
+    if (e != hipSuccess) {
+      mk_set_error("gemm: cannot reserve %d B of LDS: %s", LDS, hipGetErrorString(e));
+      return MK_ERR_LAUNCH;
+    }
+    attr_done = true;
+  }
+  GemmParams p = p0;
+  const long long r = body_rows;
+  p.M = p0.M - body_rows;
+  p.A = (const T*)p0.A + r * p0.lda;
+  p.xh = (T*)p0.xh + r * p0.ldxs;
+  p.xl = (T*)p0.xl + r * p0.ldxs;
+  if (p0.stats_out) p.stats_out = p0.stats_out + r * p0.nslot_out * 2;
+  if (p0.ln_shift_in) p.ln_shift_in = p0.ln_shift_in + r;
+  if (p0.out_f32) p.out_f32 = p0.out_f32 + r * p0.ldc;
+  const int ntm = (p.M + 191) / 192, ntn = (p.N + 255) / 256;
+  hipLaunchKernelGGL((gemm_pp_tail_kernel<T, KIND, 6>), dim3(ntm * ntn, 1, 1), dim3(512), LDS, st, p, band_m);
+  MK_CHECK_LAUNCH();
+  return MK_OK;
+}
+
 template <typename T, int AMODE, int KIND>
 int launch_k(const GemmParams& p, int groups, hipStream_t st, int band_m) {
   const int ntm = (p.M + 255) / 256, ntn = (p.N + 255) / 256;
@@ -412,7 +100,18 @@
     const int nk = p.K / BK, grid = num_cus() & ~7;
     const bool ok = groups == 1 && p.npass <= 1 && (nk & 1) == 0 && nk >= 4 && grid >= 8 && ntm * ntn > grid &&
                     !(KIND == 1 && p.ln_stats && p.ln_nslot != 16);
-    if (g_pp64_persist != 1 && ok && !(g_pp64_persist == 2 && KIND == 1)) return launch_k2<T, AMODE, KIND, true>(p, groups, st, band_m, grid);
+    if (g_pp64_persist != 1 && ok && !(g_pp64_persist == 2 && KIND == 1)) {
+      if constexpr (KIND == 2 || KIND == 3) {
+        const TailPlan tp = g_pp64_tail && p.epi == MK_EPI_LS_RESIDUAL ? plan_tail(p.M, p.N, grid) : TailPlan{p.M, 0, 0};
+        if (tp.tail_bm == 192) {
+          GemmParams pb = p;
+          pb.M = tp.body_rows;
+          const int rc = launch_k2<T, AMODE, KIND, true>(pb, groups, st, band_m, grid);
+          return rc != MK_OK ? rc : launch_tail<T, KIND>(p, tp.body_rows, st, band_m);
+        }
+      }
+      return launch_k2<T, AMODE, KIND, true>(p, groups, st, band_m, grid);
+    }
   }
   return launch_k2<T, AMODE, KIND, false>(p, groups, st, band_m, ntm * ntn);
 }
diff --git a/mickey_amd/csrc/mk_gemm_pp64_body.hpp b/mickey_amd/csrc/mk_gemm_pp64_body.hpp
--- /dev/null
+++ b/mickey_amd/csrc/mk_gemm_pp64_body.hpp
@@ -0,0 +1,373 @@
+  static_assert(WMF == 8 || (AMODE == A_DENSE && (KIND == 2 || KIND == 3) && !PERSIST && !SP && (WMF == 6 || WMF == 4 || WMF == 2)),
+                "short-row tiles: dense producers, one tile per workgroup");
+  static_assert(!SP2 || SP, "SP2 is a form of the split-operand kernel");
+  static_assert(!PERSIST || AMODE == A_DENSE, "the persistent tile loop is built for dense operands");
+  static_assert(!SP || (KIND == 0 && !PERSIST && sizeof(T) == 2), "split operands: plain epilogues, one tile per workgroup");
+  constexpr int BKA = SP ? BK / 2 : BK;
+  using V8 = typename Lp<T>::V8;
+  constexpr int BM = 32 * WMF, BN = 256;
+  constexpr int AP = WMF / 2, RPH = 16 * WMF;
+  constexpr int A_BYTES = 256 * 128, STAGE_BYTES = (256 + BN) * 128;
+  constexpr int LN_STAGE_OFF = 2 * STAGE_BYTES + 256 * 8;
+  extern __shared__ __attribute__((aligned(16))) char smem[];
+
+  const int tid0 = threadIdx.x;
+  const int wave = __builtin_amdgcn_readfirstlane(tid0 >> 6);
+  int lane = tid0 & 63, tid = tid0;
+  auto refresh_lane = [&]() {
+    if constexpr (PERSIST) {
+      asm volatile("v_mbcnt_lo_u32_b32 %0, -1, 0\n\tv_mbcnt_hi_u32_b32 %0, -1, %0" : "=v"(lane));
+      tid = wave * 64 + lane;
+    }
+  };
+  const int wm = wave >> 2, wn = wave & 3;
+  const int g = blockIdx.y;
+  const int ntm = (p.M + BM - 1) / BM, ntn = (p.N + BN - 1) / BN;
+  const int nk = p.K / BK;
+
+  const T* A = (const T*)p.A + (long long)g * p.strideA_g;
+  const T* A2 = p.A2 ? (const T*)p.A2 + (long long)g * p.strideA2_g : nullptr;
+  const T* W = (const T*)p.W + (long long)g * p.strideW_g;
+  int srow = lane >> 3, sp = lane & 7;
+  const int ntiles = ntm * ntn;
+  auto tile_origin = [&](int id, int& mm, int& nn) {
+    int tm, tn;
+    pp_tile_coords(xcd_remap(id, ntiles), ntm, ntn, band_m, tm, tn);
+    mm = tm * BM;
+    nn = tn * BN;
+  };
+  int bid = blockIdx.x;
+  int m0, n0;
+  tile_origin(bid, m0, n0);
+  unsigned woff[4], aoff[AP], aoff2[AP];
+  auto set_woff = [&](int nn0) {
+#pragma unroll
+    for (int j = 0; j < 4; ++j) {
+      const int rw = (wave * 4 + j) * 8 + srow;
+      int n = nn0 + rw;
+      n = n < p.N ? n : p.N - 1;
+      woff[j] = ((unsigned)n * (unsigned)p.ldw + swz8(rw, sp) * 8) * (unsigned)sizeof(T);
+    }
+  };
+  auto set_aoff = [&](int mm0) {
+#pragma unroll
+    for (int j = 0; j < AP; ++j) {
+      const int ra = wm * 128 + (wn * AP + j) * 8 + srow;
+      int m = WMF == 8 ? mm0 + ra : mm0 + wm * RPH + (wn * AP + j) * 8 + srow;
+      m = m < p.M ? m : p.M - 1;
+      const int c = swz8(ra, sp);
+      const unsigned cc = SP ? (unsigned)(c & 3) : (unsigned)c;
+      const bool lo = SP && (c >> 2) != 0;
+      const unsigned pb1 = !SP ? 0u : (lo ? p.pl1[1] : p.pl1[0]), pb2 = !SP ? 0u : (lo ? p.pl2[1] : p.pl2[0]);
+      if (AMODE == A_DENSE) {
+        aoff[j] = ((unsigned)m * (unsigned)p.lda + cc * 8) * (unsigned)sizeof(T) + pb1;
+        aoff2[j] = 0;
+      } else {
+        const unsigned br = (unsigned)bordered_row(m, p.H, p.Wd);
+        aoff[j] = (br * (unsigned)p.C1 + cc * 8) * (unsigned)sizeof(T) + pb1;
+        aoff2[j] = (br * (unsigned)p.C2 + cc * 8) * (unsigned)sizeof(T) + pb2;
+      }
+    }
+  };
+  set_woff(n0);
+  set_aoff(m0);
+  auto dma_w1 = [&](int s, int j) {
+    glds16_sv(W + s * BK, woff[j], smem + (s & 1) * STAGE_BYTES + A_BYTES + (wave * 4 + j) * 1024);
+  };
+  const int ntap = A2 ? 10 : 9;
+  const T* cbase = AMODE == A_DENSE ? A : A - (long long)(p.Wd + 2) * p.C1;
+  int cleft = p.C1, ctap = 0;
+  auto conv_advance = [&]() {
+    cleft -= BKA;
+    const bool wrap = cleft == 0;
+    ctap += wrap ? 1 : 0;
+    const int ty = (ctap * 11) >> 5, tx = ctap - 3 * ty;
+    const T* tapbase = ctap < 9 ? A + (long long)((ty - 1) * (p.Wd + 1) + tx - 1) * p.C1 : A2;
+    cbase = wrap ? tapbase : cbase + BKA;
+    cleft = wrap ? (ctap < 9 ? p.C1 : p.C2) : cleft;
+  };
+  auto dma_a1 = [&](int s, int j) {
+    char* dst = smem + (s & 1) * STAGE_BYTES + (wm * 16 + wn * AP + j) * 1024;
+    if (AMODE == A_DENSE) {
+      glds16_sv(A + s * BKA, aoff[j], dst);
+    } else {
+      glds16_sv(cbase, ctap < 9 ? aoff[j] : aoff2[j], dst);
+    }
+  };
+  auto dma_w = [&](int s) {
+#pragma unroll
+    for (int j = 0; j < 4; ++j) dma_w1(s, j);
+  };
+  auto dma_a = [&](int s) {
+#pragma unroll
+    for (int j = 0; j < AP; ++j) dma_a1(s, j);
+    if (AMODE != A_DENSE) conv_advance();
+  };
+
+  int fr = lane & 15, fg = lane >> 4;
+  auto derive_lane = [&]() {
+    srow = lane >> 3;
+    sp = lane & 7;
+    fr = lane & 15;
+    fg = lane >> 4;
+  };
+  auto load_w = [&](V8* wf, int par, int h) {
+    const char* sW = smem + par * STAGE_BYTES + A_BYTES;
+#pragma unroll
+    for (int i = 0; i < 4; ++i) {
+      const int rw = wn * 64 + i * 16 + fr;
+      wf[i] = *(const V8*)(sW + rw * 128 + swz8(rw, h * 4 + fg) * 16);
+    }
+  };
+  auto load_x = [&](V8* xf, int par, int h) {
+    const char* sA = smem + par * STAGE_BYTES;
+#pragma unroll
+    for (int i = 0; i < WMF; ++i) {
+      const int rx = wm * 128 + i * 16 + fr;
+      xf[i] = *(const V8*)(sA + rx * 128 + swz8(rx, h * 4 + fg) * 16);
+    }
+  };
+  auto load_frags = [&](V8* wf, V8* xf, int par, int h) {
+    load_w(wf, par, h);
+    load_x(xf, par, h);
+  };
+  f32x4 acc[WMF][4];
+  auto zero_acc = [&]() {
+#pragma unroll
+    for (int i = 0; i < WMF; ++i)
+#pragma unroll
+      for (int j = 0; j < 4; ++j) acc[i][j] = f32x4{0.f, 0.f, 0.f, 0.f};
+  };
+  if constexpr (!PERSIST) zero_acc();
+  auto mfma32 = [&](const V8* wf, const V8* xf, auto dma, int s, auto first) {
+    constexpr bool DMA = decltype(dma)::value;
+    constexpr bool FIRST = decltype(first)::value;
+    __builtin_amdgcn_s_setprio(1);
+    __builtin_amdgcn_sched_barrier(0);
+#pragma unroll
+    for (int q = 0; q < 4 * WMF; ++q) {
+      const int mi = q >> 2, ni = q & 3;
+      acc[mi][ni] = Lp<T>::mma16(wf[ni], xf[mi], FIRST ? f32x4{0.f, 0.f, 0.f, 0.f} : acc[mi][ni]);
+      if (DMA && (q & 7) == 3) {
+        __builtin_amdgcn_sched_barrier(0);
+        dma_a1(s, q >> 3);
+        __builtin_amdgcn_sched_barrier(0);
+      }
+    }
+    __builtin_amdgcn_sched_barrier(0);
+    __builtin_amdgcn_s_setprio(0);
+    if (DMA && AMODE != A_DENSE) conv_advance();
+  };
+  auto bar = [&]() {
+    asm volatile("s_waitcnt lgkmcnt(0)" ::: "memory");
+    __builtin_amdgcn_s_barrier();
+  };
+  using Yes = std::integral_constant<bool, true>;
+  using No = std::integral_constant<bool, false>;
+  V8 wf[4], xf[WMF];
+  V8 wfl[SP ? 4 : 1];
+  auto stage0 = [&](int kt, auto next1, auto next2, int sw, int sa, auto first) {
+    if constexpr (SP && SP2) {
+      bar();
+      load_frags(wf, xf, kt & 1, 0);
+      if constexpr (decltype(next1)::value) dma_w(sw);
+      bar();
+      mfma32(wf, xf, No{}, 0, first);
+      bar();
+      load_w(wf, kt & 1, 1);
+      bar();
+      mfma32(wf, xf, next2, sa, No{});
+      if constexpr (decltype(next2)::value)
+        asm volatile("s_waitcnt vmcnt(%0)" ::"n"(AP) : "memory");
+      else
+        asm volatile("s_waitcnt vmcnt(0)" ::: "memory");
+      return;
+    }
+    if constexpr (SP) {
+      bar();
+      load_frags(wf, xf, kt & 1, 0);
+      bar();
+      mfma32(wf, xf, No{}, 0, first);
+      bar();
+      load_w(wfl, kt & 1, 1);
+      if constexpr (decltype(next1)::value) dma_w(sw);
+      bar();
+      mfma32(wfl, xf, No{}, 0, No{});
+      bar();
+      load_x(xf, kt & 1, 1);
+      bar();
+      mfma32(wf, xf, next2, sa, No{});
+      if constexpr (decltype(next2)::value)
+        asm volatile("s_waitcnt vmcnt(%0)" ::"n"(AP) : "memory");
+      else
+        asm volatile("s_waitcnt vmcnt(0)" ::: "memory");
+      return;
+    }
+    bar();
+    load_frags(wf, xf, kt & 1, 0);
+    if constexpr (decltype(next1)::value) dma_w(sw);
+    bar();
+    mfma32(wf, xf, No{}, 0, first);
+    bar();
+    load_frags(wf, xf, kt & 1, 1);
+    bar();
+    mfma32(wf, xf, next2, sa, No{});
+    if constexpr (decltype(next2)::value)
+      asm volatile("s_waitcnt vmcnt(%0)" ::"n"(AP) : "memory");
+    else
+      asm volatile("s_waitcnt vmcnt(0)" ::: "memory");
+  };
+  auto stage1 = [&](int kt, auto next1, auto next2, int sw, int sa, auto first) {
+    if constexpr (SP && SP2) {
+      bar();
+      load_frags(wf, xf, kt & 1, 0);
+      if constexpr (decltype(next1)::value) dma_w(sw);
+      bar();
+      mfma32(wf, xf, No{}, 0, first);
+      bar();
+      load_w(wf, kt & 1, 1);
+      asm volatile("s_waitcnt vmcnt(0)" ::: "memory");
+      bar();
+      mfma32(wf, xf, next2, sa, No{});
+      return;
+    }
+    if constexpr (SP) {
+      bar();
+      load_frags(wf, xf, kt & 1, 0);
+      bar();
+      mfma32(wf, xf, No{}, 0, first);
+      bar();
+      load_w(wfl, kt & 1, 1);
+      if constexpr (decltype(next1)::value) dma_w(sw);
+      bar();
+      mfma32(wfl, xf, No{}, 0, No{});
+      bar();
+      load_x(xf, kt & 1, 1);
+      asm volatile("s_waitcnt vmcnt(0)" ::: "memory");
+      bar();
+      mfma32(wf, xf, next2, sa, No{});
+      return;
+    }
+    bar();
+    load_frags(wf, xf, kt & 1, 0);
+    if constexpr (decltype(next1)::value) dma_w(sw);
+    bar();
+    mfma32(wf, xf, No{}, 0, first);
+    bar();
+    load_frags(wf, xf, kt & 1, 1);
+    asm volatile("s_waitcnt vmcnt(0)" ::: "memory");
+    bar();
+    mfma32(wf, xf, next2, sa, No{});
+  };
+
+  const bool ln = KIND == 1 && p.ln_stats != nullptr;
+#if defined(MK_LN_ABL) && MK_LN_ABL == 1
+  const bool ln_fast = false && ln;
+#define MK_LN_NO_SLOW 1
+#else
+  const bool ln_fast = ln && p.ln_nslot == 16;
+#endif
+  LnRowLoads16 lnl;
+  if (ln_fast) lnl.issue(p, m0, tid);
+  constexpr bool PRODUCER = AMODE == A_DENSE && (KIND == 2 || KIND == 3);
+  ShiftLoad shl;
+  if constexpr (PRODUCER) shl.issue(p, m0, tid, 256, RPH);
+  dma_a(0);
+  dma_w(0);
+  if constexpr (!PERSIST) dma_a(1);
+  constexpr int YOUNGER = PERSIST ? 4 + AP : 4 + 2 * AP;
+  const bool publish = ln && p.ln_shift_out != nullptr && n0 == 0;
+  if (ln_fast) lnl.template finish<YOUNGER>(p, tid, (float2*)(smem + 2 * STAGE_BYTES), m0, publish);
+#ifndef MK_LN_NO_SLOW
+  else if (ln) ln_params_to_lds<256, 512>(p, m0, tid, (float2*)(smem + 2 * STAGE_BYTES), publish);
+#endif
+  if constexpr (PRODUCER) shl.template finish<YOUNGER>(tid, 256, (float*)(smem + 2 * STAGE_BYTES));
+  if constexpr (!PERSIST) asm volatile("s_waitcnt vmcnt(%0)" ::"n"(AP) : "memory");
+  const int bstep = PERSIST ? (int)gridDim.x : 0;
+  for (;;) {
+    const int nbid = bid + bstep;
+    const bool has_next = PERSIST && nbid < ntiles;
+    int m1 = m0, n1 = n0;
+    if (PERSIST && has_next) tile_origin(nbid, m1, n1);
+    if constexpr (PERSIST) {
+      refresh_lane();
+      derive_lane();
+      set_aoff(m0);
+      set_woff(n0);
+      dma_a(1);
+      if (bid == (int)blockIdx.x) asm volatile("s_waitcnt vmcnt(%0)" ::"n"(AP) : "memory");
+    }
+    bool ln_pending = false;
+    auto first_stage_done = [&]() {
+      if constexpr (PERSIST) {
+        if (ln_pending) {
+          const bool publish1 = ln && p.ln_shift_out != nullptr && n0 == 0;
+          if (ln_fast) {
+            LnRowDma16::finish<0>(p, wave, lane, (float2*)(smem + 2 * STAGE_BYTES), smem + LN_STAGE_OFF, m0, publish1);
+            asm volatile("s_waitcnt lgkmcnt(0)" ::: "memory");
+            LnRowDma16::issue<2>(p, m0, wave, lane, smem + LN_STAGE_OFF);
+          }
+          if constexpr (PRODUCER) shl.template finish<-1>(tid, 256, (float*)(smem + 2 * STAGE_BYTES));
+        }
+      }
+    };
+    auto second_stage_done = [&]() {
+      if constexpr (PERSIST) {
+        if (ln_pending && ln_fast)
+          LnRowDma16::finish<2>(p, wave, lane, (float2*)(smem + 2 * STAGE_BYTES), smem + LN_STAGE_OFF, m0,
+                                ln && p.ln_shift_out != nullptr && n0 == 0);
+      }
+    };
+    ln_pending = PERSIST && bid != (int)blockIdx.x;
+    int kt0 = 0;
+    if (wm == 0) {
+      if constexpr (PERSIST) {
+        stage0(0, Yes{}, Yes{}, 1, 2, Yes{});
+        first_stage_done();
+        stage0(1, Yes{}, Yes{}, 2, 3, No{});
+        second_stage_done();
+        kt0 = 2;
+      }
+      for (int kt = kt0; kt < nk - 2; ++kt) stage0(kt, Yes{}, Yes{}, kt + 1, kt + 2, No{});
+      if constexpr (PERSIST) {
+        set_aoff(m1);
+        stage0(nk - 2, Yes{}, Yes{}, nk - 1, 0, No{});
+        set_woff(n1);
+        stage0(nk - 1, Yes{}, No{}, 0, 0, No{});
+      } else {
+        stage0(nk - 2, Yes{}, No{}, nk - 1, 0, No{});
+        stage0(nk - 1, No{}, No{}, 0, 0, No{});
+      }
+      bar();
+    } else {
+      bar();
+      if constexpr (PERSIST) {
+        stage1(0, Yes{}, Yes{}, 1, 2, Yes{});
+        first_stage_done();
+        stage1(1, Yes{}, Yes{}, 2, 3, No{});
+        second_stage_done();
+        kt0 = 2;
+      }
+      for (int kt = kt0; kt < nk - 2; ++kt) stage1(kt, Yes{}, Yes{}, kt + 1, kt + 2, No{});
+      if constexpr (PERSIST) {
+        set_aoff(m1);
+        stage1(nk - 2, Yes{}, Yes{}, nk - 1, 0, No{});
+        set_woff(n1);
+        stage1(nk - 1, Yes{}, No{}, 0, 0, No{});
+      } else {
+        stage1(nk - 2, Yes{}, No{}, nk - 1, 0, No{});
+        stage1(nk - 1, No{}, No{}, 0, 0, No{});
+      }
+    }
+    char* wl0 = smem + STAGE_BYTES + wave * 4096;
+    refresh_lane();
+    epilogue_lds<T, KIND, AMODE == A_CONV3, 256, WMF>(p, acc, wl0, wl0 + A_BYTES, m0, n0, wm, wn, lane, g, (const float2*)(smem + 2 * STAGE_BYTES));
+    if (!(PERSIST && has_next)) break;
+    bid = nbid;
+    m0 = m1;
+    n0 = n1;
+    asm volatile("" : "+s"(m0), "+s"(n0));
+    refresh_lane();
+    if (ln_fast) LnRowDma16::issue<0>(p, m0, wave, lane, smem + LN_STAGE_OFF);
+    if constexpr (PRODUCER) shl.issue(p, m0, tid, 256, RPH);
+  }
diff --git a/mickey_amd/ops.py b/mickey_amd/ops.py
--- a/mickey_amd/ops.py
+++ b/mickey_amd/ops.py
@@ -26,6 +26,13 @@
 
 def gemm_set_tile(mode):
     call("mk_gemm_set_tile", int(mode))
+
+
+def gemm_tail_plan(M, N, cus):
+    import ctypes
+    out = (ctypes.c_int * 3)()
+    call("mk_dev_gemm_tail_plan", int(M), int(N), int(cus), ctypes.addressof(out))
+    return tuple(out)
 
 
 def gemm(a, w, bias=None, act=ACT_NONE, out_f32=False, out=None, lda=None, K=None):
```
